# microsoft/CryptoNets

Measured on AMD Instinct MI355X. Metric: encrypted images/sec (CryptoNets-MNIST, N=8192), higher is better.
Workload: dtype u64

## Files before the change

### cryptonets_amd/csrc/cn_gemm_plan.h

```cpp
#pragma once
#include "cn_policy.h"
#include <algorithm>
#include <cstdio>
#include <cstdlib>
#include <cstring>
#include <map>
#include <type_traits>
#include <unordered_map>
#include <vector>

struct GemmSwitches { bool f64, gemm_mfma, gemm_pair, digit_mfma, digit_i32; };
static const int GEMM_ERR_ARG = -1;
struct GemmRefusal {
    int rc = 0; char msg[96] = {0};
    explicit operator bool() const { return rc != 0; }
};
inline GemmRefusal gemm_refuse(const char *text) { GemmRefusal r; r.rc = GEMM_ERR_ARG; snprintf(r.msg, sizeof r.msg, "%s", text); return r; }
inline size_t gemm_al(size_t b) { return (b + 255) & ~(size_t)255; }
static const uint32_t GEMM_NONE = 0xffffffffu;

inline uint64_t gemm_abs_weight(const DevConsts &hc, uint64_t w) { return w >= hc.t_half ? hc.t.q - w : w; }
inline uint64_t lift_scalar(const DevConsts &hc, uint64_t w, uint32_t j) { return w >= hc.t_half ? w + hc.lift_inc[j] : w; }
inline bool gemm_weights_small(const DevConsts &hc, const uint64_t *W, size_t count) {
    for (size_t x = 0; x < count; x++) if (gemm_abs_weight(hc, W[x]) >> 20) return false;
    return true;
}
struct GemmArith { bool small, two; uint32_t lazy; int bits; };
inline GemmArith gemm_arith(const DevConsts &hc, const GemmSwitches &sw, bool weights_small) {
    const CnModRange qr = cn_mod_range(hc, 0, hc.k);
    const int bits = qr.bits;
    GemmArith g;
    g.bits = bits;
    g.small = weights_small && sw.f64 && bits <= 49;
    g.two = qr.light;
    if (g.small) g.lazy = g.two ? 1024u : 32768u;
    else g.lazy = (2 * bits >= 127) ? 1u : (uint32_t)std::min<uint64_t>(1u << 20, 1ull << (127 - 2 * bits));
    return g;
}
inline bool gemm_mfma_ok(const DevConsts &hc, const GemmSwitches &sw, const GemmArith &ar, uint32_t M, uint32_t K) {
    return sw.gemm_mfma && ar.small && ar.bits <= 46 && M >= 16 && (uint64_t)K * 3 < (1u << 17) && !(hc.n & 31);
}
inline uint32_t gemm_weight_planes(const DevConsts &hc, const uint64_t *W, size_t count) {
    uint64_t amax = 0;
    for (size_t x = 0; x < count; x++) amax = std::max(amax, gemm_abs_weight(hc, W[x]));
    return amax <= 127 ? 1u : (amax <= 32639 ? 2u : 3u);
}

template <class KEY> inline std::map<std::vector<KEY>, std::vector<uint32_t>> gemm_outputs_by_list(const KEY *keys, uint32_t O, uint32_t K) {
    std::map<std::vector<KEY>, std::vector<uint32_t>> groups;
    for (uint32_t o = 0; o < O; o++) groups[std::vector<KEY>(keys + (size_t)o * K, keys + (size_t)(o + 1) * K)].push_back(o);
    return groups;
}
inline bool pair_gather_lists(uint32_t O, uint32_t &K, std::vector<int32_t> &gidx, const uint64_t *W, std::vector<uint64_t> &W2) {
    if (K > 64 || O < 2) return false;
    const auto groups = gemm_outputs_by_list(gidx.data(), O, K);
    const size_t G = groups.size();
    if (G < 2 || G > 65536) return false;
    struct L { std::vector<int32_t> in; const std::vector<uint32_t> *outs; const std::vector<int32_t> *list; int32_t mate = -1; };
    std::vector<L> ls; ls.reserve(G);
    for (auto &kv : groups) {
        if (kv.second.size() > 5) return false;
        L l; l.outs = &kv.second; l.list = &kv.first;
        for (int32_t id : kv.first) if (id >= 0) l.in.push_back(id);
        std::sort(l.in.begin(), l.in.end());
        if (std::adjacent_find(l.in.begin(), l.in.end()) != l.in.end()) return false;
        ls.push_back(std::move(l));
    }
    std::unordered_map<int32_t, std::vector<uint32_t>> where;
    for (uint32_t i = 0; i < G; i++) for (int32_t id : ls[i].in) where[id].push_back(i);
    bool any = false;
    std::vector<uint32_t> cnt(G, 0), touched;
    for (uint32_t i = 0; i < G; i++) {
        if (ls[i].mate >= 0) continue;
        touched.clear();
        for (int32_t id : ls[i].in) for (uint32_t j : where[id]) if (j > i && ls[j].mate < 0) { if (!cnt[j]++) touched.push_back(j); }
        uint32_t best = 0; int32_t bj = -1;
        for (uint32_t j : touched) { if (cnt[j] > best || (cnt[j] == best && (int32_t)j < bj)) { best = cnt[j]; bj = (int32_t)j; } cnt[j] = 0; }
        if (bj >= 0 && 2 * best >= std::min(ls[i].in.size(), ls[bj].in.size()) && ls[i].in.size() + ls[bj].in.size() - best <= 64) { ls[i].mate = bj; ls[bj].mate = (int32_t)i; any = true; }
    }
    if (!any) return false;
    std::vector<std::vector<int32_t>> uni(G);
    uint32_t K2 = 0;
    for (uint32_t i = 0; i < G; i++) {
        const int32_t m = ls[i].mate;
        if (m >= 0 && (uint32_t)m < i) { uni[i] = uni[m]; continue; }
        for (int32_t id : *ls[i].list) if (id >= 0) uni[i].push_back(id);
        if (m >= 0) for (int32_t id : *ls[m].list) if (id >= 0 && !std::binary_search(ls[i].in.begin(), ls[i].in.end(), id)) uni[i].push_back(id);
        K2 = std::max<uint32_t>(K2, (uint32_t)uni[i].size());
    }
    std::vector<int32_t> g2((size_t)O * K2, -1);
    W2.assign((size_t)O * K2, 0);
    for (uint32_t i = 0; i < G; i++) {
        std::unordered_map<int32_t, uint32_t> pos;
        for (uint32_t x = 0; x < uni[i].size(); x++) pos[uni[i][x]] = x;
        for (uint32_t o : *ls[i].outs) {
            for (uint32_t x = 0; x < uni[i].size(); x++) g2[(size_t)o * K2 + x] = uni[i][x];
            for (uint32_t kk = 0; kk < K; kk++) { const int32_t id = gidx[(size_t)o * K + kk]; if (id >= 0) W2[(size_t)o * K2 + pos[id]] = W[(size_t)o * K + kk]; }
        }
    }
    gidx.swap(g2); K = K2;
    return true;
}

template <class KEY> struct GemmGroups {
    static constexpr KEY PAD = std::is_signed<KEY>::value ? (KEY)-1 : (KEY)0;
    uint32_t O = 0, G = 0, M = 0, K = 0, Kp = 0;
    bool mfma = false;
    std::vector<KEY> rows;
    std::vector<uint32_t> member;
    const uint64_t *W = nullptr;
    bool tap(uint32_t g, uint32_t kk) const { return rows[(size_t)g * Kp + kk] > PAD; }
    const uint64_t *row(uint32_t g, uint32_t m) const { const uint32_t o = member[(size_t)g * M + m]; return o == GEMM_NONE ? nullptr : W + (size_t)o * K; }
    uint64_t weight(uint32_t g, const uint64_t *wr, uint32_t kk) const { return tap(g, kk) ? wr[kk] : 0; }
};
template <class KEY> inline GemmGroups<KEY> gemm_group(const DevConsts &hc, const GemmSwitches &sw, const GemmArith &ar, const KEY *keys, const uint64_t *W, uint32_t O, uint32_t K) {
    const auto groups = gemm_outputs_by_list(keys, O, K);
    GemmGroups<KEY> gr;
    gr.O = O; gr.G = (uint32_t)groups.size(); gr.K = K; gr.W = W;
    for (auto &g : groups) gr.M = std::max<uint32_t>(gr.M, (uint32_t)g.second.size());
    gr.mfma = gemm_mfma_ok(hc, sw, ar, gr.M, K);
    gr.Kp = gr.mfma ? ((K + 31) / 32) * 32 : ((K + 15) & ~15u) + 16;
    gr.rows.assign((size_t)gr.G * gr.Kp, GemmGroups<KEY>::PAD);
    gr.member.assign((size_t)gr.G * gr.M, GEMM_NONE);
    uint32_t g = 0;
    for (auto &kv : groups) {
        memcpy(&gr.rows[(size_t)g * gr.Kp], kv.first.data(), (size_t)K * sizeof(KEY));
        for (uint32_t m = 0; m < kv.second.size(); m++) gr.member[(size_t)g * gr.M + m] = kv.second[m];
        g++;
    }
    return gr;
}

template <class KEY> inline void pack_gemm_f64(const DevConsts &hc, const GemmGroups<KEY> &gr, uint32_t tile, uint32_t rows, std::vector<char> &bytes) {
    const uint32_t mt = (gr.M + tile - 1) / tile;
    bytes.assign((size_t)gr.G * mt * rows * tile * sizeof(double), 0);
    double *tab = (double *)bytes.data();
    for (uint32_t g = 0; g < gr.G; g++) for (uint32_t m = 0; m < gr.M; m++) {
        const uint64_t *wr = gr.row(g, m);
        if (!wr) continue;
        double *dst = &tab[(((size_t)g * mt + m / tile) * rows) * tile + m % tile];
        for (uint32_t kk = 0; kk < gr.K; kk++) { const uint64_t w = gr.weight(g, wr, kk); dst[(size_t)kk * tile] = w >= hc.t_half ? -(double)(hc.t.q - w) : (double)w; }
    }
}
template <class KEY> inline void pack_gemm_int(const DevConsts &hc, const GemmGroups<KEY> &gr, uint32_t tile, std::vector<char> &bytes) {
    const uint32_t mt = (gr.M + tile - 1) / tile, K = gr.K;
    bytes.assign((size_t)hc.k * gr.G * mt * K * tile * sizeof(uint64_t), 0);
    uint64_t *tab = (uint64_t *)bytes.data();
    for (uint32_t j = 0; j < hc.k; j++) for (uint32_t g = 0; g < gr.G; g++) for (uint32_t m = 0; m < gr.M; m++) {
        const uint64_t *wr = gr.row(g, m);
        if (!wr) continue;
        uint64_t *dst = &tab[((((size_t)j * gr.G + g) * mt + m / tile) * K) * tile + m % tile];
        for (uint32_t kk = 0; kk < K; kk++) { const uint64_t w = gr.weight(g, wr, kk); dst[(size_t)kk * tile] = w ? lift_scalar(hc, w, j) : 0; }
    }
}
template <class KEY> inline void pack_gemm_mfma(const DevConsts &hc, const GemmGroups<KEY> &gr, uint32_t P, std::vector<char> &wbytes) {
    const uint32_t mtiles = (gr.M + 31) / 32, ksteps = (gr.K + 31) / 32;
    const uint64_t t = hc.t.q;
    wbytes.assign((size_t)gr.G * P * mtiles * ksteps * 1024, 0);
    for (uint32_t g = 0; g < gr.G; g++) for (uint32_t m = 0; m < gr.M; m++) {
        const uint64_t *wr = gr.row(g, m);
        if (!wr) continue;
        const uint32_t mt = m / 32, r = m % 32;
        for (uint32_t kk = 0; kk < gr.K; kk++) {
            const uint64_t w = gr.weight(g, wr, kk);
            if (!w) continue;
            const int64_t sw = w >= hc.t_half ? -(int64_t)(t - w) : (int64_t)w;
            const uint32_t rec = ((uint32_t)(sw + 0x808080) ^ 0x808080u);
            const uint32_t ks = kk / 32, half = (kk % 32) / 16, tt = kk % 16;
            for (uint32_t p = 0; p < P; p++)
                wbytes[((((size_t)g * P + p) * mtiles + mt) * ksteps + ks) * 1024 + (size_t)(half * 32 + r) * 16 + tt] = (char)(uint8_t)(rec >> (8 * p));
        }
    }
}
template <class KEY> inline uint64_t gemm_row_sum_max(const DevConsts &hc, const GemmGroups<KEY> &gr, uint64_t stop) {
    uint64_t sum_max = 0;
    for (uint32_t g = 0; g < gr.G; g++) for (uint32_t m = 0; m < gr.M; m++) {
        const uint64_t *wr = gr.row(g, m);
        if (!wr) continue;
        uint64_t sum = 0;
        for (uint32_t kk = 0; kk < gr.K; kk++) if (gr.tap(g, kk)) { sum += gemm_abs_weight(hc, wr[kk]); if (sum > stop) return stop + 1; }
        sum_max = std::max(sum_max, sum);
    }
    return sum_max;
}
template <class KEY> inline bool gemm_one_limb(const DevConsts &hc, const GemmArith &ar, const GemmGroups<KEY> &gr) {
    static const bool on = !(getenv("CN_GEMM_ONE_LIMB") && !atoi(getenv("CN_GEMM_ONE_LIMB")));
    if (!on || !ar.small || ar.bits > 49 || gr.K > ar.lazy) return false;
    const uint64_t room = (1ull << 53) / cn_mod_range(hc, 0, hc.k).qmax;
    return room && gemm_row_sum_max(hc, gr, room - 1) <= room - 1;
}
template <class KEY> inline void gemm_form_and_pack(const DevConsts &hc, const GemmArith &ar, const GemmGroups<KEY> &gr, GemmLayout &L, std::vector<char> &wbytes) {
    const uint32_t M = gr.M;
    L.K = gr.K; L.Kp = gr.Kp; L.G = gr.G; L.M = M; L.small = ar.small; L.two = ar.two; L.lazy = ar.lazy; L.mfma = gr.mfma;
    if (gr.mfma) {
        L.P = gemm_weight_planes(hc, gr.W, (size_t)gr.O * gr.K); L.mtiles = (M + 31) / 32; L.ksteps = (gr.K + 31) / 32;
        pack_gemm_mfma(hc, gr, L.P, wbytes);
    } else if (ar.small) {
        L.MT = M >= 16 ? 20 : (M >= 8 ? 10 : (M >= 3 ? 5 : 1));
        pack_gemm_f64(hc, gr, L.MT, gemm_f64_rows(gr.K), wbytes);
        L.one = gemm_one_limb(hc, ar, gr);
    } else {
        L.MT = M >= 8 ? 10 : (M >= 3 ? 5 : 1);
        pack_gemm_int(hc, gr, L.MT, wbytes);
    }
}
template <class KEY> inline void gemm_digit_form(const DevConsts &hc, const GemmSwitches &sw, const GemmGroups<KEY> &gr, GemmLayout &L, std::vector<char> &dbytes) {
    if (!L.small || hc.k < 2 || hc.dbc < 1 || hc.dbc > 30) return;
    uint64_t qmin = ~0ull; for (uint32_t j = 0; j < hc.k; j++) qmin = std::min(qmin, hc.q[j].q);
    const uint64_t dmax = (1ull << hc.dbc) - 1, lim = std::min<uint64_t>((qmin - 1) / 2, (1ull << 52) - 1) / dmax;
    const uint64_t sum_max = gemm_row_sum_max(hc, gr, lim);
    if (sum_max > lim) return;
    L.dig = true; L.sum_abs_w = sum_max; L.dig_mfma = L.mfma && sw.digit_mfma && hc.dbc <= 14 && !(hc.n & 255); L.dig_i32 = sw.digit_i32 && cn_digit_sum_fits_i32(sum_max, hc.dbc);
    if (L.dig_mfma) return;
    L.dMT = digit_gemm_tile(L.M); L.dKw = digit_gemm_rows(L.K);
    pack_gemm_f64(hc, gr, L.dMT, L.dKw, dbytes);
}

template <class E> inline void gemm_assemble(const std::vector<E> &gather, const std::vector<E> &outs, const std::vector<E> &bias, const std::vector<char> &wbytes,
                                             const std::vector<char> &dbytes, GemmLayout &L, std::vector<char> &image) {
    L.off_oidx = gemm_al(gather.size() * sizeof(E)); L.off_bidx = L.off_oidx + gemm_al(outs.size() * sizeof(E)); L.off_w = L.off_bidx + gemm_al(bias.size() * sizeof(E));
    L.off_dw = L.off_w + gemm_al(wbytes.size());
    image.assign(L.off_dw + gemm_al(dbytes.size()), 0);
    if (!gather.empty()) memcpy(image.data(), gather.data(), gather.size() * sizeof(E));
    if (!outs.empty()) memcpy(image.data() + L.off_oidx, outs.data(), outs.size() * sizeof(E));
    if (!bias.empty()) memcpy(image.data() + L.off_bidx, bias.data(), bias.size() * sizeof(E));
    if (!wbytes.empty()) memcpy(image.data() + L.off_w, wbytes.data(), wbytes.size());
    if (!dbytes.empty()) memcpy(image.data() + L.off_dw, dbytes.data(), dbytes.size());
}

inline GemmRefusal gemm_plan_indices(const DevConsts &hc, const GemmSwitches &sw, const int32_t *idx, const uint64_t *W, uint32_t O, uint32_t K, const int32_t *bias_idx,
                                     uint32_t bias_count, GemmLayout &L, std::vector<char> &image, uint32_t &max_in, uint64_t &nnz) {
    if (!O || !K || !W) return gemm_refuse("empty scalar GEMM");
    std::vector<int32_t> gidx((size_t)O * K);
    for (uint32_t o = 0; o < O; o++) {
        bool any = false;
        for (uint32_t kk = 0; kk < K; kk++) {
            const int32_t id = idx ? idx[(size_t)o * K + kk] : (int32_t)kk;
            const uint64_t w = W[(size_t)o * K + kk];
            if (w >= hc.t.q) return gemm_refuse("weight >= plain modulus");
            if (id >= 0) max_in = std::max<uint32_t>(max_in, (uint32_t)id + 1);
            if (id >= 0 && w) { any = true; nnz++; }
            gidx[(size_t)o * K + kk] = id;
        }
        if (!any) { GemmRefusal r = gemm_refuse(""); snprintf(r.msg, sizeof r.msg, "output %u has no non-zero term (AddMany of nothing)", o); return r; }
        if (bias_idx && (bias_idx[o] < 0 || (uint32_t)bias_idx[o] >= bias_count)) return gemm_refuse("bias index out of range");
    }
    const GemmArith ar = gemm_arith(hc, sw, gemm_weights_small(hc, W, (size_t)O * K));
    std::vector<uint64_t> W2;
    if (sw.gemm_pair && ar.small && pair_gather_lists(O, K, gidx, W, W2)) W = W2.data();
    const GemmGroups<int32_t> gr = gemm_group(hc, sw, ar, gidx.data(), W, O, K);
    std::vector<int32_t> hoidx(gr.member.size(), -1), hbidx(gr.member.size(), 0);
    for (size_t x = 0; x < gr.member.size(); x++) if (gr.member[x] != GEMM_NONE) { hoidx[x] = (int32_t)gr.member[x]; if (bias_idx) hbidx[x] = bias_idx[gr.member[x]]; }
    std::vector<char> wbytes, dbytes;
    gemm_form_and_pack(hc, ar, gr, L, wbytes);
    gemm_digit_form(hc, sw, gr, L, dbytes);
    gemm_assemble(gr.rows, hoidx, hbidx, wbytes, dbytes, L, image);
    return GemmRefusal();
}
struct GemmAddressPlan {
    GemmLayout L; std::vector<char> image;
    bool abs = false, any_bias = false;
    uint64_t ibase = ~0ull, obase = ~0ull, bbase = ~0ull;
    uint64_t some_input = 0;
};
inline void gemm_plan_addresses(const DevConsts &hc, const GemmSwitches &sw, const uint64_t *A, const uint64_t *W, const uint64_t *out, const uint64_t *bias, uint32_t O, uint32_t K,
                                bool rel_on, GemmAddressPlan &R) {
    const GemmArith ar = gemm_arith(hc, sw, gemm_weights_small(hc, W, (size_t)O * K));
    const GemmGroups<uint64_t> gr = gemm_group(hc, sw, ar, A, W, O, K);
    std::vector<uint64_t> hoidx(gr.member.size(), 0), hbidx(gr.member.size(), 0);
    bool all_bias = true;
    for (size_t x = 0; x < gr.member.size(); x++) if (gr.member[x] != GEMM_NONE) {
        hoidx[x] = out[gr.member[x]]; hbidx[x] = bias[gr.member[x]];
        R.any_bias = R.any_bias || hbidx[x]; all_bias = all_bias && hbidx[x];
    }
    for (uint64_t a : gr.rows) if (a && !R.some_input) R.some_input = a;
    std::vector<char> wbytes;
    gemm_form_and_pack(hc, ar, gr, R.L, wbytes);
    bool rel = rel_on && (!R.any_bias || all_bias);
    if (rel) {
        for (uint64_t a : gr.rows) if (a) R.ibase = std::min(R.ibase, a);
        for (uint64_t a : hoidx) if (a) R.obase = std::min(R.obase, a);
        for (uint64_t a : hbidx) if (a) R.bbase = std::min(R.bbase, a);
        auto fits = [](uint64_t a, uint64_t base) { return !a || (((a - base) & 255) == 0 && ((a - base) >> 8) < 0x7fffffffull); };
        for (uint64_t a : gr.rows) rel = rel && fits(a, R.ibase);
        for (uint64_t a : hoidx) rel = rel && fits(a, R.obase);
        for (uint64_t a : hbidx) rel = rel && fits(a, R.bbase);
        rel = rel && R.ibase != ~0ull && R.obase != ~0ull;
    }
    R.abs = !rel;
    if (R.abs) { gemm_assemble(gr.rows, hoidx, hbidx, wbytes, {}, R.L, R.image); return; }
    auto relative = [](const std::vector<uint64_t> &a, uint64_t base, int32_t none) {
        std::vector<int32_t> r(a.size(), none);
        for (size_t x = 0; x < a.size(); x++) if (a[x]) r[x] = (int32_t)((a[x] - base) >> 8);
        return r;
    };
    gemm_assemble(relative(gr.rows, R.ibase, -1), relative(hoidx, R.obase, -1), relative(hbidx, R.bbase, 0), wbytes, {}, R.L, R.image);
}
```

### cryptonets_amd/csrc/cn_k_gemm.hip.h

```cpp
#pragma once
#include "cn_dev_common.hip.h"

DEV void gemm_block_coords(uint32_t bx, uint32_t by, uint32_t chunks, uint32_t limbs, uint32_t mtiles, uint32_t G, uint32_t &chunk, uint32_t &limb, uint32_t &mt, uint32_t &g,
                           uint32_t order = 0) {
    if (order == 1) {
        const uint32_t x = bx & 7, r = bx >> 3;
        if (mtiles == 1) { mt = 0; g = r; } else { mt = r % mtiles; g = r / mtiles; }
        const uint32_t sl = by * 8 + x;
        chunk = sl & (chunks - 1); limb = sl >> (__ffs((int)chunks) - 1);
        return;
    }
    const uint32_t b = bx, D = chunks * limbs * G;
    uint32_t d;
    if ((D & 7) == 0) { const uint32_t r = b >> 3; mt = r % mtiles; d = (r / mtiles) * 8 + (b & 7); }
    else { d = b % D; mt = b / D; }
    chunk = d % chunks; limb = (d / chunks) % limbs; g = d / (chunks * limbs);
}
DEV const NTT_GLOBAL uint64_t *gmem(uint64_t a) { return (const NTT_GLOBAL uint64_t *)a; }
DEV NTT_GLOBAL uint64_t *gmem_w(uint64_t a) { return (NTT_GLOBAL uint64_t *)a; }
struct GemmUnits { uint32_t in, out, bias; };
template <bool ABS> struct GemmTab { typedef int32_t T; };
template <> struct GemmTab<true> { typedef uint64_t T; };
template <int MT, bool ABS = false>
__global__ void __launch_bounds__(256) k_scalar_gemm(const uint64_t *__restrict__ in, const void *__restrict__ idx_, const uint64_t *__restrict__ Wl,
                                                     const void *__restrict__ out_idx_, const uint64_t *__restrict__ bias, const void *__restrict__ bias_idx_,
                                                     uint64_t *__restrict__ out, const DevConsts *__restrict__ C, uint32_t chunks, uint32_t G, uint32_t M,
                                                     uint32_t K, uint32_t mtiles, uint32_t lazy, uint32_t Kp, uint32_t obase, uint32_t polys, uint32_t order, GemmUnits U) {
    typedef typename GemmTab<ABS>::T TT;
    const TT *idx = (const TT *)idx_, *out_idx = (const TT *)out_idx_, *bias_idx = (const TT *)bias_idx_;
    const uint32_t n = C->n, k = C->k, limbs = polys * k;
    uint32_t chunk, limb, mt, g;
    gemm_block_coords(blockIdx.x, blockIdx.y, chunks, limbs, mtiles, G, chunk, limb, mt, g, order);
    const uint32_t j = limb % k, i = chunk * blockDim.x + threadIdx.x;
    const size_t ctw = (size_t)limbs * n, e = (size_t)limb * n + i;
    const size_t iu = U.in ? U.in : ctw, ou = U.out ? U.out : ctw, bu = U.bias ? U.bias : n;
    const DMod qm = C->q[j];
    u128 acc[MT];
#pragma unroll
    for (int m = 0; m < MT; m++) acc[m] = 0;
    const TT *gi = idx + (size_t)g * Kp;
    const uint64_t *gw = Wl + (((size_t)j * G + g) * mtiles + mt) * (size_t)K * MT;
    const uint32_t mcnt = min((uint32_t)MT, M - mt * MT);
    for (uint32_t k0 = 0; k0 < K; k0 += lazy) {
        const uint32_t k1 = min(K, k0 + lazy);
        for (uint32_t kk = k0; kk < k1; kk++) {
            uint64_t x;
            if constexpr (ABS) { const uint64_t a = gi[kk]; if (!a) continue; x = gmem(a)[e]; }
            else { const int32_t id = gi[kk]; if (id < 0) continue; x = in[(size_t)id * iu + e]; }
#pragma unroll
            for (int m = 0; m < MT; m++) acc[m] += (u128)x * gw[(size_t)kk * MT + m];
        }
        if (k1 < K) {
#pragma unroll
            for (int m = 0; m < MT; m++) acc[m] = bred128(acc[m], qm);
        }
    }
#pragma unroll
    for (int m = 0; m < MT; m++) {
        const uint32_t o = g * M + mt * MT + m;
        if constexpr (ABS) {
            if ((uint32_t)m < mcnt && out_idx[o]) {
                uint64_t r = bred128(acc[m], qm);
                if (bias_idx && bias_idx[o] && limb < k) { const uint64_t bv = gmem(bias_idx[o])[i]; if (bv) r = addmod(r, scale_plain(C, bv, j), qm.q); }
                gmem_w(out_idx[o])[e] = r;
            }
        } else if ((uint32_t)m < mcnt && out_idx[o] >= 0) {
            uint64_t r = bred128(acc[m], qm);
            if (bias && limb < k) { const uint64_t bv = bias[(size_t)bias_idx[o] * bu + i]; if (bv) r = addmod(r, scale_plain(C, bv, j), qm.q); }
            out[(size_t)(obase + (uint32_t)out_idx[o]) * ou + e] = r;
        }
    }
}

#ifndef GEMM_DPP_W
#define GEMM_DPP_W 1
#endif
template <int NL, int LW> DEV double gemm_limb(uint64_t x, int l) {
    if constexpr (NL == 1) return BzF::from_u64(x & 0x000FFFFFFFFFFFFFull);
    else return (double)(uint32_t)(l == NL - 1 ? x >> (l * LW) : (x >> (l * LW)) & ((1ull << LW) - 1));
}
template <int LANE> DEV void fmac_bcast(double &acc, double w, double x) {
    asm volatile("v_fmac_f64_dpp %0, %1, %2 row_newbcast:%3 row_mask:0xf bank_mask:0xf" : "+v"(acc) : "v"(w), "v"(x), "n"(LANE));
}
DEV void fmac_bcast_lane(int lane, double &acc, double w, double x) {
    switch (lane) {
    case 0: fmac_bcast<0>(acc, w, x); break;   case 1: fmac_bcast<1>(acc, w, x); break;   case 2: fmac_bcast<2>(acc, w, x); break;   case 3: fmac_bcast<3>(acc, w, x); break;
    case 4: fmac_bcast<4>(acc, w, x); break;   case 5: fmac_bcast<5>(acc, w, x); break;   case 6: fmac_bcast<6>(acc, w, x); break;   case 7: fmac_bcast<7>(acc, w, x); break;
    case 8: fmac_bcast<8>(acc, w, x); break;   case 9: fmac_bcast<9>(acc, w, x); break;   case 10: fmac_bcast<10>(acc, w, x); break; case 11: fmac_bcast<11>(acc, w, x); break;
    case 12: fmac_bcast<12>(acc, w, x); break; case 13: fmac_bcast<13>(acc, w, x); break; case 14: fmac_bcast<14>(acc, w, x); break; default: fmac_bcast<15>(acc, w, x); break;
    }
}
template <int MT, int NL, int LW, bool ABS = false>
__global__ void __launch_bounds__(256) k_scalar_gemm_f64(const uint64_t *__restrict__ in, const void *__restrict__ idx_, const double *__restrict__ Wd,
                                                         const void *__restrict__ out_idx_, const uint64_t *__restrict__ bias, const void *__restrict__ bias_idx_,
                                                         uint64_t *__restrict__ out, const DevConsts *__restrict__ C, uint32_t chunks, uint32_t G, uint32_t M,
                                                         uint32_t K, uint32_t mtiles, uint32_t lazy, uint32_t Kp, uint32_t obase, uint32_t polys, uint32_t order, uint32_t Kw, GemmUnits U) {
    typedef typename GemmTab<ABS>::T TT;
    const TT *idx = (const TT *)idx_, *out_idx = (const TT *)out_idx_, *bias_idx = (const TT *)bias_idx_;
    const uint32_t n = C->n, k = C->k, limbs = polys * k;
    uint32_t chunk, limb, mt, g;
    gemm_block_coords(blockIdx.x, blockIdx.y, chunks, limbs, mtiles, G, chunk, limb, mt, g, order);
    const uint32_t j = limb % k, i = chunk * blockDim.x + threadIdx.x;
    const size_t ctw = (size_t)limbs * n, e = (size_t)limb * n + i;
    const size_t iu = U.in ? U.in : ctw, ou = U.out ? U.out : ctw, bu = U.bias ? U.bias : n;
    const DMod qm = C->q[j];
    double acc[NL][MT], res[MT];
#pragma unroll
    for (int m = 0; m < MT; m++) {
        res[m] = 0.0;
#pragma unroll
        for (int l = 0; l < NL; l++) acc[l][m] = 0.0;
    }
    const TT *gi = idx + (size_t)g * Kp;
    const double *gw = Wd + ((size_t)g * mtiles + mt) * (size_t)Kw * MT;
    const uint32_t mcnt = min((uint32_t)MT, M - mt * MT);
    const BzF::Mod mq = {C->qd[j], C->qinvd[j]};
    auto fold = [&]() {
#pragma unroll
        for (int m = 0; m < MT; m++) {
            double r = acc[NL - 1][m];
            acc[NL - 1][m] = 0.0;
#pragma unroll
            for (int l = NL - 2; l >= 0; l--) { r = __dadd_rn(BzF::mulmod(r, (double)(1u << LW), mq), acc[l][m]); acc[l][m] = 0.0; }
            res[m] = BzF::center(__dadd_rn(res[m], r), mq);
        }
    };
#ifndef GEMM_PF_SMALL
#define GEMM_PF_SMALL 4
#endif
    constexpr int PF = (MT <= 5) ? GEMM_PF_SMALL : 4;
    static_assert(PF % 4 == 0, "gather indices travel in 16 B scalar loads of four");
    auto fetch = [&](uint64_t (&x)[PF], uint32_t kk) {
        const uint32_t kc = min(kk, Kp - PF);
        if constexpr (ABS) {
#pragma unroll
            for (int c = 0; c < PF; c += 4) {
                const ulonglong2 a01 = *reinterpret_cast<const ulonglong2 *>(__builtin_assume_aligned(gi + kc + c, 16));
                const ulonglong2 a23 = *reinterpret_cast<const ulonglong2 *>(__builtin_assume_aligned(gi + kc + c + 2, 16));
                const uint64_t ad[4] = {a01.x, a01.y, a23.x, a23.y};
#pragma unroll
                for (int p = 0; p < 4; p++) x[c + p] = gmem(ad[p] ? ad[p] : (uint64_t)in)[e];
            }
        } else {
#pragma unroll
            for (int c = 0; c < PF; c += 4) {
                const int4 ids = *reinterpret_cast<const int4 *>(__builtin_assume_aligned(gi + kc + c, 16));
                const int32_t id[4] = {ids.x, ids.y, ids.z, ids.w};
#pragma unroll
                for (int p = 0; p < 4; p++) x[c + p] = in[(size_t)max(id[p], 0) * iu + e];
            }
        }
    };
    constexpr int WB = MT >= 20 ? 1 : (MT * PF <= 20 ? PF : 20 / MT);
    constexpr bool WSET = WB == PF;
    auto wload = [&](double (&w)[WB * MT], uint32_t kk) {
        const double *wp = gw + (size_t)kk * MT;
#pragma unroll
        for (int q = 0; q < WB * MT; q++) w[q] = wp[q];
    };
    auto terms = [&](const uint64_t (&x)[PF], uint32_t kk, const double (&w0)[WB * MT]) {
#pragma unroll
        for (int p0 = 0; p0 < PF; p0 += WB) {
            double w[WB * MT];
            if constexpr (WSET) {
#pragma unroll
                for (int q = 0; q < WB * MT; q++) w[q] = w0[q];
            } else wload(w, kk + p0);
#pragma unroll
            for (int p = p0; p < p0 + WB; p++) {
                double xl[NL];
#pragma unroll
                for (int l = 0; l < NL; l++) xl[l] = gemm_limb<NL, LW>(x[p], l);
#pragma unroll
                for (int m = 0; m < MT; m++) {
#pragma unroll
                    for (int l = 0; l < NL; l++) acc[l][m] = __fma_rn(xl[l], w[(p - p0) * MT + m], acc[l][m]);
                }
            }
        }
    };
    constexpr bool DPPW = GEMM_DPP_W && MT == 20 && PF == 4;
    constexpr int WV = DPPW ? PF * MT / 16 : 1;
    auto wfetch = [&](double (&wv)[WV], uint32_t kk) {
        const double *wp = gw + (size_t)min(kk, K + 4) * MT + (threadIdx.x & 15);
#pragma unroll
        for (int v = 0; v < WV; v++) wv[v] = wp[16 * v];
    };
    auto terms_dpp = [&](const uint64_t (&x)[PF], double (&wv)[WV]) {
#pragma unroll
        for (int p = 0; p < PF; p++) {
            double xl[NL];
#pragma unroll
            for (int l = 0; l < NL; l++) xl[l] = gemm_limb<NL, LW>(x[p], l);
            asm volatile("s_nop 1");
#pragma unroll
            for (int m = 0; m < MT; m++) {
                const int f = p * MT + m;
#pragma unroll
                for (int l = 0; l < NL; l++) fmac_bcast_lane(f & 15, acc[l][m], wv[(f >> 4) % WV], xl[l]);
            }
        }
    };
    for (uint32_t k0 = 0; k0 < K; k0 += lazy) {
        const uint32_t k1 = min(K, k0 + lazy);
        uint64_t xa[PF], xb[PF];
        if constexpr (DPPW) {
            double wa[WV], wb[WV];
            fetch(xa, k0); wfetch(wa, k0);
            for (uint32_t kk = k0; kk < k1; kk += 2 * PF) {
                fetch(xb, kk + PF); wfetch(wb, kk + PF);
                terms_dpp(xa, wa);
                fetch(xa, kk + 2 * PF); wfetch(wa, kk + 2 * PF);
                terms_dpp(xb, wb);
            }
        } else {
            const uint32_t sets = (k1 - k0 + PF - 1) / PF;
            uint32_t kk = k0;
            double wa[WB * MT], wb[WB * MT];
            fetch(xa, k0);
            for (uint32_t it = sets >> 1; it; it--, kk += 2 * PF) {
                if constexpr (WSET) { wload(wa, kk); __builtin_amdgcn_sched_barrier(0); }
                fetch(xb, kk + PF);
                terms(xa, kk, wa);
                if constexpr (WSET) { wload(wb, kk + PF); __builtin_amdgcn_sched_barrier(0); }
                fetch(xa, kk + 2 * PF);
                terms(xb, kk + PF, wb);
            }
            if (sets & 1) { if constexpr (WSET) wload(wa, kk); terms(xa, kk, wa); }
        }
        fold();
    }
    constexpr int OB = MT < 5 ? MT : 5;
    const uint32_t olast = G * M - 1;
    const bool hb = (ABS ? bias_idx != nullptr : bias != nullptr) && limb < k;
#pragma unroll
    for (int m0 = 0; m0 < MT; m0 += OB) {
        uint32_t oo[OB];
        TT oi[OB], bi[OB];
        bool st[OB];
        uint64_t bv[OB];
#pragma unroll
        for (int u = 0; u < OB; u++) oo[u] = min(g * M + mt * MT + m0 + u, olast);
#pragma unroll
        for (int u = 0; u < OB; u++) { oi[u] = out_idx[oo[u]]; bi[u] = 0; bv[u] = 0; }
        if (hb) {
#pragma unroll
            for (int u = 0; u < OB; u++) bi[u] = bias_idx[oo[u]];
        }
#pragma unroll
        for (int u = 0; u < OB; u++) st[u] = (uint32_t)(m0 + u) < mcnt && (ABS ? oi[u] != 0 : (int64_t)oi[u] >= 0);
        if (hb) {
#pragma unroll
            for (int u = 0; u < OB; u++) {
                if constexpr (ABS) bv[u] = gmem(st[u] && bi[u] ? bi[u] : (uint64_t)in)[i];
                else bv[u] = bias[(size_t)(st[u] ? bi[u] : (TT)0) * bu + i];
            }
#pragma unroll
            for (int u = 0; u < OB; u++) if (!(st[u] && (ABS ? bi[u] != 0 : true))) bv[u] = 0;
        }
#pragma unroll
        for (int u = 0; u < OB; u++) {
            if (!st[u]) continue;
            const double rc = res[m0 + u] < 0.0 ? __dadd_rn(res[m0 + u], mq.q) : res[m0 + u];
            uint64_t r = (uint64_t)__double_as_longlong(__dadd_rn(rc, 4503599627370496.0)) & 0x000FFFFFFFFFFFFFull;
            if (bv[u]) r = addmod(r, scale_plain(C, bv[u], j), qm.q);
            if constexpr (ABS) gmem_w(oi[u])[e] = r;
            else out[(size_t)(obase + (uint32_t)oi[u]) * ou + e] = r;
        }
    }
}

typedef int v4i_t __attribute__((ext_vector_type(4)));
typedef int v16i_t __attribute__((ext_vector_type(16)));
DEV uint32_t byte_perm(uint32_t hi, uint32_t lo, uint32_t sel) { return __builtin_amdgcn_perm(hi, lo, sel); }
#ifndef GEMM_MFMA_DEPTH
#define GEMM_MFMA_DEPTH 2
#endif
enum { GEMM_CT = 0, GEMM_BSK = 1, GEMM_Y = 2 };
struct GemmBskForm { static constexpr int form = GEMM_BSK; };
struct GemmYForm { static constexpr int form = GEMM_Y; };
template <int P, bool ABS, class... FORM_>
__global__ void __launch_bounds__(256, 2) k_scalar_gemm_mfma(const uint64_t *__restrict__ in, const void *__restrict__ idx_, const int8_t *__restrict__ Wf,
                                                             const void *__restrict__ out_idx_, const uint64_t *__restrict__ bias, const void *__restrict__ bias_idx_,
                                                             uint64_t *__restrict__ out, const DevConsts *__restrict__ C, uint32_t G, uint32_t M, uint32_t mtiles,
                                                             uint32_t ksteps, uint32_t obase, uint32_t polys, GemmUnits U) {
    constexpr int FORM = (GEMM_CT + ... + FORM_::form);
    static_assert(sizeof...(FORM_) <= 1 && (FORM == GEMM_CT || !ABS), "the pre-floor forms use relative addressing");
    typedef typename GemmTab<ABS>::T TT;
    const TT *idx = (const TT *)idx_, *out_idx = (const TT *)out_idx_, *bias_idx = (const TT *)bias_idx_;
    constexpr int ND = FORM == GEMM_BSK ? 7 : 6, D = ND + P - 1, NB = GEMM_MFMA_DEPTH + 1;
    __shared__ __align__(16) uint32_t frag[NB][ND][64][4];
    const uint32_t n = C->n, k = FORM == GEMM_BSK ? C->kb : C->k, limbs = polys * k, ctiles = n >> 5;
    const uint32_t lane = threadIdx.x & 63, wave = (uint32_t)__builtin_amdgcn_readfirstlane((int)(threadIdx.x >> 6)), half = lane >> 5, col = lane & 31;
    uint32_t b = blockIdx.x;
    const uint32_t ctile = b % ctiles; b /= ctiles;
    const uint32_t limb = b % limbs; b /= limbs;
    const uint32_t mgroups = (mtiles + 3) >> 2, mg = b % mgroups, g = b / mgroups;
    const uint32_t mt = mg * 4 + wave;
    const bool active = mt < mtiles;
    const uint32_t j = limb % k;
    const size_t ctw = (size_t)limbs * n, e = (size_t)limb * n + (size_t)ctile * 32 + col;
    const size_t iu = U.in ? U.in : ctw, ou = U.out ? U.out : ctw, bu = U.bias ? U.bias : n;
    const uint32_t Kp = ksteps * 32;
    const TT *gi = idx + (size_t)g * Kp + 4 * wave;
    const int8_t *wf = Wf + ((((size_t)g * P) * mtiles + (active ? mt : 0)) * ksteps) * 1024 + (size_t)lane * 16;
    v16i_t acc[D];
#pragma unroll
    for (int d = 0; d < D; d++)
#pragma unroll
        for (int r = 0; r < 16; r++) acc[d][r] = 0;
    const uint64_t BIAS = FORM == GEMM_BSK ? 0x0080808080808080ull : 0x0000808080808080ull;
    const uint32_t klast = ksteps - 1;
    auto load_idx = [&](TT (&s)[8], uint32_t ks) {
        const TT *t = gi + (size_t)min(ks, klast) * 32;
#pragma unroll
        for (int u = 0; u < 4; u++) { s[u] = t[u]; s[4 + u] = t[16 + u]; }
    };
    auto load_x = [&](uint64_t (&x)[4], const TT (&s)[8]) {
#pragma unroll
        for (int u = 0; u < 4; u++) {
            if constexpr (ABS) {
                const uint64_t a0 = s[u] ? s[u] : (uint64_t)in, a1 = s[4 + u] ? s[4 + u] : (uint64_t)in;
                x[u] = gmem(half ? a1 : a0)[e];
            } else {
                size_t o0 = (size_t)max(s[u], 0) * iu, o1 = (size_t)max(s[4 + u], 0) * iu;
                asm volatile("" : "+s"(o0), "+s"(o1));
                x[u] = in[(half ? o1 : o0) + e];
            }
        }
    };
    auto load_a = [&](v4i_t (&af)[P], uint32_t ks) {
#pragma unroll
        for (int p = 0; p < P; p++) af[p] = *reinterpret_cast<const v4i_t *>(wf + ((size_t)p * mtiles * ksteps + min(ks, klast)) * 1024);
    };
    uint64_t xs[NB][4];
    v4i_t afs[NB][P];
    TT nidx[8];
    load_idx(nidx, 0);
#pragma unroll
    for (int s = 0; s < GEMM_MFMA_DEPTH; s++) { load_x(xs[s], nidx); load_a(afs[s], s); load_idx(nidx, s + 1); }
    auto step = [&](uint64_t (&x)[4], v4i_t (&af)[P], uint64_t (&xn)[4], v4i_t (&afn)[P], uint32_t ks, uint32_t (*fb)[64][4]) {
        uint32_t lo[4], hi[4];
#pragma unroll
        for (int u = 0; u < 4; u++) {
            uint64_t xw = x[u];
            if constexpr (FORM == GEMM_Y) {
                const BzF::Mod mq = {C->qd[j], C->qinvd[j]};
                const double yv = bz_canon(BzF::mulmod(lazy_value(xw), C->bd.fl_c1n_q[j], mq), mq);
                xw = (uint64_t)__double_as_longlong(__dadd_rn(yv, 4503599627370496.0)) & 0x000FFFFFFFFFFFFFull;
            }
            const uint64_t y = (xw + BIAS) ^ BIAS; lo[u] = (uint32_t)y; hi[u] = (uint32_t)(y >> 32);
        }
        const uint32_t ab02 = byte_perm(lo[1], lo[0], 0x06020400u), cd02 = byte_perm(lo[3], lo[2], 0x06020400u);
        const uint32_t ab13 = byte_perm(lo[1], lo[0], 0x07030501u), cd13 = byte_perm(lo[3], lo[2], 0x07030501u);
        const uint32_t hab = byte_perm(hi[1], hi[0], 0x05010400u), hcd = byte_perm(hi[3], hi[2], 0x05010400u);
        fb[0][lane][wave] = byte_perm(cd02, ab02, 0x05040100u);
        fb[1][lane][wave] = byte_perm(cd13, ab13, 0x05040100u);
        fb[2][lane][wave] = byte_perm(cd02, ab02, 0x07060302u);
        fb[3][lane][wave] = byte_perm(cd13, ab13, 0x07060302u);
        fb[4][lane][wave] = byte_perm(hcd, hab, 0x05040100u);
        fb[5][lane][wave] = byte_perm(hcd, hab, 0x07060302u);
        if constexpr (ND == 7) {
            const uint32_t hab6 = byte_perm(hi[1], hi[0], 0x06020602u), hcd6 = byte_perm(hi[3], hi[2], 0x06020602u);
            fb[ND - 1][lane][wave] = byte_perm(hcd6, hab6, 0x05040100u);
        }
        load_x(xn, nidx); load_a(afn, ks + GEMM_MFMA_DEPTH);
        load_idx(nidx, ks + GEMM_MFMA_DEPTH + 1);
        __syncthreads();
        if (active) {
            v4i_t bf[ND];
#pragma unroll
            for (int i = 0; i < ND; i++) bf[i] = *reinterpret_cast<const v4i_t *>(&fb[i][lane][0]);
#pragma unroll
            for (int p = 0; p < P; p++)
#pragma unroll
                for (int i = 0; i < ND; i++) acc[i + p] = __builtin_amdgcn_mfma_i32_32x32x32_i8(af[p], bf[i], acc[i + p], 0, 0, 0);
        }
    };
    uint32_t ks = 0;
    for (; ks + NB <= ksteps; ks += NB) {
#pragma unroll
        for (int s = 0; s < NB; s++) step(xs[s], afs[s], xs[(s + GEMM_MFMA_DEPTH) % NB], afs[(s + GEMM_MFMA_DEPTH) % NB], ks + s, frag[s]);
    }
#pragma unroll
    for (int s = 0; s < NB - 1; s++)
        if (ks + s < ksteps) step(xs[s], afs[s], xs[(s + GEMM_MFMA_DEPTH) % NB], afs[(s + GEMM_MFMA_DEPTH) % NB], ks + s, frag[s]);
    if (!active) return;
    if constexpr (FORM == GEMM_Y) {
#pragma unroll
        for (int r = 0; r < 16; r++) {
            const uint32_t row = (uint32_t)(r & 3) + 8u * (uint32_t)(r >> 2) + 4u * half, o = g * M + mt * 32 + row;
            if (mt * 32 + row >= M) continue;
            uint64_t v = 0;
#pragma unroll
            for (int d = 0; d < D; d++) v += (uint64_t)(int64_t)acc[d][r] << (8 * d);
            if (out_idx[o] < 0) continue;
            out[(size_t)(obase + (uint32_t)out_idx[o]) * ou + e] = v;
        }
        return;
    }
    const uint32_t jm = FORM == GEMM_BSK ? C->k + j : j;
    const BzF::Mod mq = {C->qd[jm], C->qinvd[jm]};
    const DMod qm = C->q[FORM == GEMM_BSK ? 0 : j];
    const double c24 = BzF::center(16777216.0, mq), c48 = BzF::center(__dmul_rn(c24, 16777216.0), mq);
#pragma unroll
    for (int r = 0; r < 16; r++) {
        const uint32_t row = (uint32_t)(r & 3) + 8u * (uint32_t)(r >> 2) + 4u * half, o = g * M + mt * 32 + row;
        if (mt * 32 + row >= M) continue;
        auto group = [&](int d0) {
            double t = (double)acc[d0][r];
            if (d0 + 1 < D) t = __fma_rn((double)acc[d0 + 1 < D ? d0 + 1 : d0][r], 256.0, t);
            if (d0 + 2 < D) t = __fma_rn((double)acc[d0 + 2 < D ? d0 + 2 : d0][r], 65536.0, t);
            return t;
        };
        double v = __dadd_rn(group(0), BzF::mulmod(group(3), c24, mq));
        if (D > 6) v = __dadd_rn(v, BzF::mulmod(group(6), c48, mq));
        uint64_t res = BzF::to_u64(v, mq);
        if constexpr (ABS) {
            if (!out_idx[o]) continue;
            if (bias_idx && bias_idx[o] && limb < k) { const uint64_t bv = gmem(bias_idx[o])[(size_t)ctile * 32 + col]; if (bv) res = addmod(res, scale_plain(C, bv, j), qm.q); }
            gmem_w(out_idx[o])[e] = res;
        } else {
            if (out_idx[o] < 0) continue;
            if (FORM == GEMM_CT && bias && limb < k) { const uint64_t bv = bias[(size_t)bias_idx[o] * bu + (size_t)ctile * 32 + col]; if (bv) res = addmod(res, scale_plain(C, bv, j), qm.q); }
            out[(size_t)(obase + (uint32_t)out_idx[o]) * ou + e] = res;
        }
    }
}

template <class... E> struct DigitWord { typedef double type; };
template <> struct DigitWord<int32_t> { typedef int32_t type; };
template <int MT, int DG, class... E>
__global__ void __launch_bounds__(256) k_digit_gemm(const uint64_t *__restrict__ in, size_t in_unit, const int32_t *__restrict__ idx, const double *__restrict__ Wd,
                                                    const int32_t *__restrict__ out_idx, typename DigitWord<E...>::type *__restrict__ S, const DevConsts *__restrict__ C, uint32_t G, uint32_t M,
                                                    uint32_t K, uint32_t mtiles, uint32_t Kp, uint32_t Kw, uint32_t ndg) {
    const uint32_t n = C->n, k = C->k, chunks = n >> 8;
    uint32_t chunk, lj, mt, g;
    gemm_block_coords(blockIdx.x, 0, chunks, k * ndg, mtiles, G, chunk, lj, mt, g);
    const uint32_t l = lj % k, d0 = (lj / k) * DG, nd = C->rl_dig[l];
    if (d0 >= nd) return;
    uint32_t g0 = 0;
    for (uint32_t x = 0; x < l; x++) g0 += C->rl_dig[x];
    const uint32_t i = chunk * 256 + threadIdx.x, dbc = (uint32_t)C->dbc, mask = (1u << dbc) - 1;
    const size_t e = (size_t)l * n + i;
    uint32_t sh[DG];
#pragma unroll
    for (int d = 0; d < DG; d++) sh[d] = min(dbc * (d0 + (uint32_t)d), 63u);
    double acc[DG][MT];
#pragma unroll
    for (int d = 0; d < DG; d++)
#pragma unroll
        for (int m = 0; m < MT; m++) acc[d][m] = 0.0;
    const int32_t *gi = idx + (size_t)g * Kp;
    const double *gw = Wd + ((size_t)g * mtiles + mt) * (size_t)Kw * MT;
    constexpr int PF = 4, WB = MT > 10 ? 1 : 2;
    auto fetch = [&](uint64_t (&x)[PF], uint32_t kk) {
        const int4 ids = *reinterpret_cast<const int4 *>(__builtin_assume_aligned(gi + min(kk, Kp - PF), 16));
        const int32_t id[4] = {ids.x, ids.y, ids.z, ids.w};
#pragma unroll
        for (int p = 0; p < PF; p++) x[p] = in[(size_t)max(id[p], 0) * in_unit + e];
    };
    auto terms = [&](const uint64_t (&x)[PF], uint32_t kk) {
#pragma unroll
        for (int p0 = 0; p0 < PF; p0 += WB) {
            double w[WB * MT];
            const double *wp = gw + (size_t)(kk + p0) * MT;
#pragma unroll
            for (int q = 0; q < WB * MT; q++) w[q] = wp[q];
#pragma unroll
            for (int p = p0; p < p0 + WB; p++) {
                double dg[DG];
#pragma unroll
                for (int d = 0; d < DG; d++) dg[d] = (double)((uint32_t)(x[p] >> sh[d]) & mask);
#pragma unroll
                for (int m = 0; m < MT; m++)
#pragma unroll
                    for (int d = 0; d < DG; d++) acc[d][m] = __fma_rn(dg[d], w[(p - p0) * MT + m], acc[d][m]);
            }
        }
    };
    {
        const uint32_t sets = (K + PF - 1) / PF;
        uint32_t kk = 0;
        uint64_t xa[PF], xb[PF];
        fetch(xa, 0);
        for (uint32_t it = sets >> 1; it; it--, kk += 2 * PF) {
            fetch(xb, kk + PF);
            terms(xa, kk);
            fetch(xa, kk + 2 * PF);
            terms(xb, kk + PF);
        }
        if (sets & 1) terms(xa, kk);
    }
    const uint32_t tot = C->rl_tot;
#pragma unroll
    for (int m = 0; m < MT; m++) {
        const uint32_t mm = mt * MT + (uint32_t)m;
        if (mm >= M) break;
        const int32_t o = out_idx[g * M + mm];
        if (o < 0) continue;
#pragma unroll
        for (int d = 0; d < DG; d++)
            if (d0 + (uint32_t)d < nd) S[((size_t)o * tot + g0 + d0 + (uint32_t)d) * n + i] = (typename DigitWord<E...>::type)acc[d][m];
    }
}

template <int P, int DG, class... E>
__global__ void __launch_bounds__(256, 2) k_digit_gemm_mfma(const uint64_t *__restrict__ in, size_t in_unit, const int32_t *__restrict__ idx, const int8_t *__restrict__ Wf,
                                                            const int32_t *__restrict__ out_idx, typename DigitWord<E...>::type *__restrict__ S, const DevConsts *__restrict__ C, uint32_t G,
                                                            uint32_t M, uint32_t mtiles, uint32_t ksteps, uint32_t ndg) {
    constexpr int NP = 2 * DG, D = P + 1, NB = GEMM_MFMA_DEPTH + 1;
    __shared__ __align__(16) uint32_t frag[NB][NP][64][4];
    const uint32_t n = C->n, k = C->k, ctiles = n >> 5;
    const uint32_t lane = threadIdx.x & 63, wave = (uint32_t)__builtin_amdgcn_readfirstlane((int)(threadIdx.x >> 6)), half = lane >> 5, col = lane & 31;
    uint32_t b = blockIdx.x;
    const uint32_t x8 = b & 7; b >>= 3;
    const uint32_t dgi = b % ndg; b /= ndg;
    const uint32_t ctile = (b % (ctiles >> 3)) * 8 + x8; b /= ctiles >> 3;
    const uint32_t l = b % k; b /= k;
    const uint32_t mgroups = (mtiles + 3) >> 2, mg = b % mgroups, g = b / mgroups;
    const uint32_t d0 = dgi * DG, nd = C->rl_dig[l];
    if (d0 >= nd) return;
    const uint32_t cnt = min((uint32_t)DG, nd - d0);
    uint32_t g0 = 0;
    for (uint32_t x = 0; x < l; x++) g0 += C->rl_dig[x];
    const uint32_t mt = mg * 4 + wave;
    const bool active = mt < mtiles;
    const uint32_t dbc = (uint32_t)C->dbc, mask = (1u << dbc) - 1;
    uint32_t sh[DG];
#pragma unroll
    for (int d = 0; d < DG; d++) sh[d] = min(dbc * (d0 + (uint32_t)d), 63u);
    const size_t e = (size_t)l * n + (size_t)ctile * 32 + col;
    const uint32_t Kp = ksteps * 32;
    const int32_t *gi = idx + (size_t)g * Kp + 4 * wave;
    const int8_t *wf = Wf + ((((size_t)g * P) * mtiles + (active ? mt : 0)) * ksteps) * 1024 + (size_t)lane * 16;
    v16i_t acc[DG][D];
#pragma unroll
    for (int d = 0; d < DG; d++)
#pragma unroll
        for (int j = 0; j < D; j++)
#pragma unroll
            for (int r = 0; r < 16; r++) acc[d][j][r] = 0;
    const uint32_t klast = ksteps - 1;
    auto load_idx = [&](int32_t (&s)[8], uint32_t ks) {
        const int32_t *t = gi + (size_t)min(ks, klast) * 32;
#pragma unroll
        for (int u = 0; u < 4; u++) { s[u] = t[u]; s[4 + u] = t[16 + u]; }
    };
    auto load_x = [&](uint64_t (&x)[4], const int32_t (&s)[8]) {
#pragma unroll
        for (int u = 0; u < 4; u++) {
            size_t o0 = (size_t)max(s[u], 0) * in_unit, o1 = (size_t)max(s[4 + u], 0) * in_unit;
            asm volatile("" : "+s"(o0), "+s"(o1));
            x[u] = in[(half ? o1 : o0) + e];
        }
    };
    auto load_a = [&](v4i_t (&af)[P], uint32_t ks) {
#pragma unroll
        for (int p = 0; p < P; p++) af[p] = *reinterpret_cast<const v4i_t *>(wf + ((size_t)p * mtiles * ksteps + min(ks, klast)) * 1024);
    };
    uint64_t xs[NB][4];
    v4i_t afs[NB][P];
    int32_t nidx[8];
    load_idx(nidx, 0);
#pragma unroll
    for (int s = 0; s < GEMM_MFMA_DEPTH; s++) { load_x(xs[s], nidx); load_a(afs[s], s); load_idx(nidx, s + 1); }
    auto step = [&](uint64_t (&x)[4], v4i_t (&af)[P], uint64_t (&xn)[4], v4i_t (&afn)[P], uint32_t ks, uint32_t (*fb)[64][4]) {
#pragma unroll
        for (int d = 0; d < DG; d++) {
            uint32_t t[4];
#pragma unroll
            for (int u = 0; u < 4; u++) t[u] = ((uint32_t)(x[u] >> sh[d]) & mask) + 128u;
            const uint32_t ab = byte_perm(t[1], t[0], 0x05010400u), cd = byte_perm(t[3], t[2], 0x05010400u);
            fb[2 * d][lane][wave] = byte_perm(cd, ab, 0x05040100u) ^ 0x80808080u;
            fb[2 * d + 1][lane][wave] = byte_perm(cd, ab, 0x07060302u);
        }
        load_x(xn, nidx); load_a(afn, ks + GEMM_MFMA_DEPTH);
        load_idx(nidx, ks + GEMM_MFMA_DEPTH + 1);
        __syncthreads();
        if (active) {
#pragma unroll
            for (int d = 0; d < DG; d++) {
                if ((uint32_t)d >= cnt) continue;
                const v4i_t blo = *reinterpret_cast<const v4i_t *>(&fb[2 * d][lane][0]), bhi = *reinterpret_cast<const v4i_t *>(&fb[2 * d + 1][lane][0]);
#pragma unroll
                for (int p = 0; p < P; p++) acc[d][p] = __builtin_amdgcn_mfma_i32_32x32x32_i8(af[p], blo, acc[d][p], 0, 0, 0);
#pragma unroll
                for (int p = 0; p < P; p++) acc[d][p + 1] = __builtin_amdgcn_mfma_i32_32x32x32_i8(af[p], bhi, acc[d][p + 1], 0, 0, 0);
            }
        }
    };
    uint32_t ks = 0;
    for (; ks + NB <= ksteps; ks += NB) {
#pragma unroll
        for (int s = 0; s < NB; s++) step(xs[s], afs[s], xs[(s + GEMM_MFMA_DEPTH) % NB], afs[(s + GEMM_MFMA_DEPTH) % NB], ks + s, frag[s]);
    }
#pragma unroll
    for (int s = 0; s < NB - 1; s++)
        if (ks + s < ksteps) step(xs[s], afs[s], xs[(s + GEMM_MFMA_DEPTH) % NB], afs[(s + GEMM_MFMA_DEPTH) % NB], ks + s, frag[s]);
    if (!active) return;
    const uint32_t tot = C->rl_tot, olast = G * M - 1;
    int32_t oo[16];
#pragma unroll
    for (int r = 0; r < 16; r++) {
        const uint32_t mm = mt * 32 + (uint32_t)(r & 3) + 8u * (uint32_t)(r >> 2) + 4u * half;
        oo[r] = out_idx[min(g * M + mm, olast)];
        if (mm >= M) oo[r] = -1;
    }
#pragma unroll
    for (int d = 0; d < DG; d++) {
        if ((uint32_t)d >= cnt) continue;
#pragma unroll
        for (int r = 0; r < 16; r++) {
            if (oo[r] < 0) continue;
            typename DigitWord<E...>::type *dst = S + ((size_t)oo[r] * tot + g0 + d0 + (uint32_t)d) * n + (size_t)ctile * 32 + col;
            if constexpr (std::is_same<typename DigitWord<E...>::type, int32_t>::value) {
                uint32_t v = (uint32_t)acc[d][D - 1][r];
#pragma unroll
                for (int j = D - 2; j >= 0; j--) v = (v << 8) + (uint32_t)acc[d][j][r];
                *dst = (int32_t)v;
            } else {
                double v = (double)acc[d][0][r];
#pragma unroll
                for (int j = 1; j < D; j++) v = __fma_rn((double)acc[d][j][r], (double)(1u << (8 * j)), v);
                *dst = v;
            }
        }
    }
}

typedef uint64_t ps_u64x2 __attribute__((ext_vector_type(2)));
typedef double ps_f64x2 __attribute__((ext_vector_type(2)));
DEV uint64_t ps_reduce(uint64_t x, const DMod &m) {
    const uint64_t r = x - __umul64hi(x, m.r1) * m.q;
    return r >= m.q ? r - m.q : r;
}
typedef int32_t ps_i32x2 __attribute__((ext_vector_type(2)));
template <int ND, class... E>
__global__ void __launch_bounds__(256) k_product_sum(const uint64_t *__restrict__ prod_, uint32_t K, uint64_t *__restrict__ out_, typename DigitWord<E...>::type *__restrict__ S_,
                                                     const DevConsts *__restrict__ C) {
    typedef const NTT_GLOBAL ps_u64x2 *In;
    constexpr int PF = 4;
    const uint32_t n = C->n, k = C->k, n2 = n >> 1, tiles = n >> 9;
    uint32_t b = blockIdx.x;
    const uint32_t tile = b % tiles; b /= tiles;
    const uint32_t l = b % k, o = b / k;
    const uint32_t p = tile * 256 + threadIdx.x;
    const uint32_t dbc = (uint32_t)C->dbc, mask = (1u << dbc) - 1, nd = C->rl_dig[l];
    uint32_t g0 = 0;
    for (uint32_t x = 0; x < l; x++) g0 += C->rl_dig[x];
    uint32_t sh[ND];
#pragma unroll
    for (int d = 0; d < ND; d++) sh[d] = min(dbc * (uint32_t)d, 63u);
    const size_t comp = (size_t)k * n2, unit = 3 * comp;
    const NTT_GLOBAL char *src = (const NTT_GLOBAL char *)prod_ + (size_t)o * K * unit * 16;
    const uint32_t lane_off = (l * n2 + p) * 16;
    uint64_t c0x = 0, c0y = 0, c1x = 0, c1y = 0, dx[ND], dy[ND];
#pragma unroll
    for (int d = 0; d < ND; d++) { dx[d] = 0; dy[d] = 0; }
    auto fetch = [&](ps_u64x2 (&x)[PF][3], uint32_t kk) {
#pragma unroll
        for (int t = 0; t < PF; t++) {
            const NTT_GLOBAL char *s = src + (size_t)min(kk + (uint32_t)t, K - 1) * unit * 16;
#pragma unroll
            for (int c = 0; c < 3; c++) x[t][c] = *(In)(s + (size_t)c * comp * 16 + lane_off);
        }
    };
    auto term = [&](const ps_u64x2 (&x)[3]) {
        c0x += x[0].x; c0y += x[0].y; c1x += x[1].x; c1y += x[1].y;
#pragma unroll
        for (int d = 0; d < ND; d++) { dx[d] += (uint32_t)(x[2].x >> sh[d]) & mask; dy[d] += (uint32_t)(x[2].y >> sh[d]) & mask; }
    };
    auto terms = [&](const ps_u64x2 (&x)[PF][3]) {
#pragma unroll
        for (int t = 0; t < PF; t++) term(x[t]);
    };
    auto tail = [&](const ps_u64x2 (&x)[PF][3], uint32_t nv) {
#pragma unroll
        for (int t = 0; t < PF; t++) if ((uint32_t)t < nv) term(x[t]);
    };
    {
        uint32_t kk = 0;
        ps_u64x2 xa[PF][3], xb[PF][3];
        fetch(xa, 0);
        for (uint32_t it = K / (2 * PF); it; it--, kk += 2 * PF) {
            fetch(xb, kk + PF);
            terms(xa);
            fetch(xa, kk + 2 * PF);
            terms(xb);
        }
        const uint32_t r = K - kk;
        if (r > PF) fetch(xb, kk + PF);
        tail(xa, min(r, (uint32_t)PF));
        if (r > PF) tail(xb, r - PF);
    }
    const DMod m = C->q[l];
    typedef NTT_GLOBAL ps_u64x2 *Out;
    Out dst = (Out)out_ + (size_t)o * 2 * comp + (size_t)l * n2 + p;
    ps_u64x2 v;
    v.x = ps_reduce(c0x, m); v.y = ps_reduce(c0y, m); dst[0] = v;
    v.x = ps_reduce(c1x, m); v.y = ps_reduce(c1y, m); dst[comp] = v;
    typedef typename DigitWord<E...>::type SE;
    typedef typename std::conditional<std::is_same<SE, int32_t>::value, ps_i32x2, ps_f64x2>::type SV;
    typedef NTT_GLOBAL SV *OutS;
    OutS sd = (OutS)S_ + ((size_t)o * C->rl_tot + g0) * n2 + p;
#pragma unroll
    for (int d = 0; d < ND; d++)
        if ((uint32_t)d < nd) { SV w; w.x = (SE)dx[d]; w.y = (SE)dy[d]; sd[(size_t)d * n2] = w; }
}
```

### cryptonets_amd/csrc/cn_l_gemm.hip

```cpp
#include "cn_runtime.h"
#include <algorithm>
#include "cn_k_gemm.hip.h"

struct GemmGrid { dim3 grid; uint32_t order; };
static GemmGrid gemm_grid(cn_ctx *c, const GemmLaunch &g, uint32_t mtiles) {
    const uint32_t slices = c->chunks * g.polys * c->hc.k;
    if (g.order == 1 && (slices & 7) == 0 && (c->chunks & (c->chunks - 1)) == 0 && (uint64_t)8 * mtiles * g.G < (1ull << 31) && slices / 8 < 65536)
        return {dim3(8 * mtiles * g.G, slices / 8), 1u};
    return {dim3((uint32_t)((size_t)slices * mtiles * g.G)), 0u};
}
template <int MT, bool ABS> static void launch_int(cn_ctx *c, const GemmLaunch &g) {
    const uint32_t mtiles = (g.M + MT - 1) / MT;
    const GemmGrid gg = gemm_grid(c, g, mtiles);
    hipLaunchKernelGGL((k_scalar_gemm<MT, ABS>), gg.grid, dim3(c->bs), 0, c->stream, g.in, g.idx, (const uint64_t *)g.W, g.oidx, g.bias, g.bidx, g.out, c->dc,
                       c->chunks, g.G, g.M, g.K, mtiles, g.lazy, g.Kp, g.obase, g.polys, gg.order, GemmUnits{g.in_unit, g.out_unit, g.bias_unit});
}
template <int MT, bool ABS> static void launch_f64(cn_ctx *c, const GemmLaunch &g) {
    const uint32_t mtiles = (g.M + MT - 1) / MT;
    const GemmGrid gg = gemm_grid(c, g, mtiles);
    if (g.one) hipLaunchKernelGGL((k_scalar_gemm_f64<MT, 1, 0, ABS>), gg.grid, dim3(c->bs), 0, c->stream, g.in, g.idx, (const double *)g.W, g.oidx, g.bias,
                                  g.bidx, g.out, c->dc, c->chunks, g.G, g.M, g.K, mtiles, g.lazy, g.Kp, g.obase, g.polys, gg.order, gemm_f64_rows(g.K), GemmUnits{g.in_unit, g.out_unit, g.bias_unit});
    else if (g.two) hipLaunchKernelGGL((k_scalar_gemm_f64<MT, 2, 22, ABS>), gg.grid, dim3(c->bs), 0, c->stream, g.in, g.idx, (const double *)g.W, g.oidx, g.bias,
                                  g.bidx, g.out, c->dc, c->chunks, g.G, g.M, g.K, mtiles, g.lazy, g.Kp, g.obase, g.polys, gg.order, gemm_f64_rows(g.K), GemmUnits{g.in_unit, g.out_unit, g.bias_unit});
    else hipLaunchKernelGGL((k_scalar_gemm_f64<MT, 3, 17, ABS>), gg.grid, dim3(c->bs), 0, c->stream, g.in, g.idx, (const double *)g.W, g.oidx, g.bias,
                            g.bidx, g.out, c->dc, c->chunks, g.G, g.M, g.K, mtiles, g.lazy, g.Kp, g.obase, g.polys, gg.order, gemm_f64_rows(g.K), GemmUnits{g.in_unit, g.out_unit, g.bias_unit});
}
template <bool ABS> static int launch(cn_ctx *c, const GemmLaunch &g) {
    if (g.small) {
        switch (g.MT) {
            case 20: launch_f64<20, ABS>(c, g); break;
            case 10: launch_f64<10, ABS>(c, g); break;
            case 5: launch_f64<5, ABS>(c, g); break;
            case 1: launch_f64<1, ABS>(c, g); break;
            default: return cn_fail(CN_ERR_ARG, "internal: scalar GEMM tile %u", g.MT);
        }
    } else {
        switch (g.MT) {
            case 10: launch_int<10, ABS>(c, g); break;
            case 5: launch_int<5, ABS>(c, g); break;
            case 1: launch_int<1, ABS>(c, g); break;
            default: return cn_fail(CN_ERR_ARG, "internal: scalar GEMM tile %u", g.MT);
        }
    }
    HIPCHK(hipGetLastError());
    cn_launch_count(c);
    return 0;
}
int cn_l_gemm(cn_ctx *c, const GemmLaunch &g) { return g.abs ? launch<true>(c, g) : launch<false>(c, g); }

template <int P, bool ABS> static void launch_mfma(cn_ctx *c, const GemmLaunch &g) {
    const uint32_t mgroups = (g.mtiles + 3) / 4;
    if constexpr (!ABS && P <= 2) {
        if (g.form) {
            const size_t pblocks = (size_t)g.G * mgroups * g.polys * (g.form == GEMM_BSK ? c->hc.kb : c->hc.k) * (c->hc.n / 32);
            if (g.form == GEMM_BSK) hipLaunchKernelGGL((k_scalar_gemm_mfma<P, false, GemmBskForm>), dim3((uint32_t)pblocks), dim3(256), 0, c->stream, g.in, g.idx, (const int8_t *)g.W, g.oidx,
                                                       nullptr, nullptr, g.out, c->dc, g.G, g.M, g.mtiles, g.ksteps, g.obase, g.polys, GemmUnits{g.in_unit, g.out_unit, 0u});
            else hipLaunchKernelGGL((k_scalar_gemm_mfma<P, false, GemmYForm>), dim3((uint32_t)pblocks), dim3(256), 0, c->stream, g.in, g.idx, (const int8_t *)g.W, g.oidx,
                                    nullptr, nullptr, g.out, c->dc, g.G, g.M, g.mtiles, g.ksteps, g.obase, g.polys, GemmUnits{g.in_unit, g.out_unit, 0u});
            return;
        }
    }
    const size_t blocks = (size_t)g.G * mgroups * g.polys * c->hc.k * (c->hc.n / 32);
    hipLaunchKernelGGL((k_scalar_gemm_mfma<P, ABS>), dim3((uint32_t)blocks), dim3(256), 0, c->stream, g.in, g.idx, (const int8_t *)g.W, g.oidx, g.bias, g.bidx, g.out,
                       c->dc, g.G, g.M, g.mtiles, g.ksteps, g.obase, g.polys, GemmUnits{g.in_unit, g.out_unit, g.bias_unit});
}
template <bool ABS> static int launch_mfma_p(cn_ctx *c, const GemmLaunch &g) {
    if (g.form && (ABS || g.P > 2 || g.form > GEMM_Y || !g.in_unit || !g.out_unit)) return cn_fail(CN_ERR_ARG, "internal: pre-floor GEMM form %u", g.form);
    switch (g.P) {
        case 1: launch_mfma<1, ABS>(c, g); break;
        case 2: launch_mfma<2, ABS>(c, g); break;
        case 3: launch_mfma<3, ABS>(c, g); break;
        default: return cn_fail(CN_ERR_ARG, "internal: %u weight digit planes", g.P);
    }
    HIPCHK(hipGetLastError());
    cn_launch_count(c);
    return 0;
}
int cn_l_gemm_mfma(cn_ctx *c, const GemmLaunch &g) { return g.abs ? launch_mfma_p<true>(c, g) : launch_mfma_p<false>(c, g); }

template <int MT> static void launch_digit(cn_ctx *c, const DigitGemmLaunch &g, uint32_t ndg, uint32_t mtiles) {
    const size_t blocks = (size_t)(c->hc.n >> 8) * c->hc.k * ndg * mtiles * g.G;
    if (g.i32) hipLaunchKernelGGL((k_digit_gemm<MT, 5, int32_t>), dim3((uint32_t)blocks), dim3(256), 0, c->stream, g.in, g.in_unit, (const int32_t *)g.idx, (const double *)g.W,
                                  (const int32_t *)g.oidx, (int32_t *)g.S, c->dc, g.G, g.M, g.K, mtiles, g.Kp, g.Kw, ndg);
    else hipLaunchKernelGGL((k_digit_gemm<MT, 5>), dim3((uint32_t)blocks), dim3(256), 0, c->stream, g.in, g.in_unit, (const int32_t *)g.idx, (const double *)g.W,
                            (const int32_t *)g.oidx, (double *)g.S, c->dc, g.G, g.M, g.K, mtiles, g.Kp, g.Kw, ndg);
}
template <int P, int DG> static void launch_digit_mfma(cn_ctx *c, const DigitGemmLaunch &g, uint32_t ndg, size_t blocks) {
    if (g.i32) hipLaunchKernelGGL((k_digit_gemm_mfma<P, DG, int32_t>), dim3((uint32_t)blocks), dim3(256), 0, c->stream, g.in, g.in_unit, (const int32_t *)g.idx, (const int8_t *)g.W,
                                  (const int32_t *)g.oidx, (int32_t *)g.S, c->dc, g.G, g.M, g.mtiles, g.ksteps, ndg);
    else hipLaunchKernelGGL((k_digit_gemm_mfma<P, DG>), dim3((uint32_t)blocks), dim3(256), 0, c->stream, g.in, g.in_unit, (const int32_t *)g.idx, (const int8_t *)g.W,
                            (const int32_t *)g.oidx, (double *)g.S, c->dc, g.G, g.M, g.mtiles, g.ksteps, ndg);
}
static int digit_gemm_mfma(cn_ctx *c, const DigitGemmLaunch &g, uint32_t ndmax) {
    const uint32_t DG = digit_gemm_mfma_group(g.P), ndg = (ndmax + DG - 1) / DG, mgroups = (g.mtiles + 3) / 4;
    const uint64_t blocks = (uint64_t)g.G * mgroups * c->hc.k * (c->hc.n / 32) * ndg;
    if ((c->hc.n & 255) || !g.ksteps || blocks >= (1ull << 31)) return cn_fail(CN_ERR_ARG, "internal: digit GEMM grid");
    switch (g.P) {
        case 1: launch_digit_mfma<1, 3>(c, g, ndg, blocks); break;
        case 2: launch_digit_mfma<2, 3>(c, g, ndg, blocks); break;
        case 3: launch_digit_mfma<3, 2>(c, g, ndg, blocks); break;
        default: return cn_fail(CN_ERR_ARG, "internal: %u weight digit planes", g.P);
    }
    HIPCHK(hipGetLastError());
    cn_launch_count(c);
    c->cnt.dg_mfma++;
    return 0;
}
int cn_l_digit_gemm(cn_ctx *c, const DigitGemmLaunch &g) {
    uint32_t ndmax = 0; for (uint32_t l = 0; l < c->hc.k; l++) ndmax = std::max(ndmax, c->hc.rl_dig[l]);
    if (g.mfma) return digit_gemm_mfma(c, g, ndmax);
    const uint32_t ndg = (ndmax + 4) / 5, mtiles = (g.M + g.MT - 1) / g.MT;
    if ((c->hc.n & 255) || (uint64_t)(c->hc.n >> 8) * c->hc.k * ndg * mtiles * g.G >= (1ull << 31)) return cn_fail(CN_ERR_ARG, "internal: digit GEMM grid");
    switch (g.MT) {
        case 10: launch_digit<10>(c, g, ndg, mtiles); break;
        case 2: launch_digit<2>(c, g, ndg, mtiles); break;
        default: return cn_fail(CN_ERR_ARG, "internal: digit GEMM tile %u", g.MT);
    }
    HIPCHK(hipGetLastError());
    cn_launch_count(c);
    return 0;
}

template <int ND> static void launch_product_sum(cn_ctx *c, const ProductSumLaunch &g, uint32_t blocks) {
    if (g.i32) hipLaunchKernelGGL((k_product_sum<ND, int32_t>), dim3(blocks), dim3(256), 0, c->stream, g.prod, g.K, g.out, (int32_t *)g.S, c->dc);
    else hipLaunchKernelGGL((k_product_sum<ND>), dim3(blocks), dim3(256), 0, c->stream, g.prod, g.K, g.out, (double *)g.S, c->dc);
}
int cn_l_product_sum(cn_ctx *c, const ProductSumLaunch &g) {
    uint32_t ndmax = 0; for (uint32_t l = 0; l < c->hc.k; l++) ndmax = std::max(ndmax, c->hc.rl_dig[l]);
    const uint64_t blocks = (uint64_t)(c->hc.n >> 9) * c->hc.k * g.outputs;
    if ((c->hc.n & 511) || !g.K || !g.outputs || ndmax > PRODUCT_SUM_MAX_DIGITS || c->hc.dbc > 31 || blocks >= (1ull << 31)) return cn_fail(CN_ERR_ARG, "internal: product sum grid");
    if (ndmax <= 2) launch_product_sum<2>(c, g, (uint32_t)blocks);
    else if (ndmax <= 4) launch_product_sum<4>(c, g, (uint32_t)blocks);
    else if (ndmax <= 5) launch_product_sum<5>(c, g, (uint32_t)blocks);
    else launch_product_sum<8>(c, g, (uint32_t)blocks);
    HIPCHK(hipGetLastError());
    cn_launch_count(c);
    return 0;
}
```

### cryptonets_amd/csrc/cn_policy.h

```cpp
#pragma once
#include "cn_internal.h"

enum { POL_U64 = 0, POL_F64 = 1, POL_F64L = 2 };

struct CnModRange {
    bool f64ok;
    bool light;
    int bits;
    uint64_t qmax;
};
inline CnModRange cn_mod_range(const DevConsts &hc, uint32_t base_off, uint32_t nmod) {
    CnModRange r{true, true, 0, 0};
    for (uint32_t m = base_off; m < base_off + nmod; m++) {
        const uint64_t q = m < hc.k ? hc.q[m].q : (m < hc.k + hc.kb ? hc.bsk[m - hc.k].q : hc.t.q);
        r.f64ok = r.f64ok && hc.f64ok[m];
        if (q > r.qmax) r.qmax = q;
    }
    r.light = !(r.qmax >> 44);
    r.bits = r.qmax ? 64 - __builtin_clzll(r.qmax) : 0;
    return r;
}
inline int cn_policy(const CnModRange &r, bool use_f64) { return !(use_f64 && r.f64ok) ? POL_U64 : (r.light ? POL_F64L : POL_F64); }
inline bool cn_digit_sum_fits_i32(uint64_t sum_abs_w, int dbc) {
    if (dbc < 1 || dbc > 31) return false;
    return (unsigned __int128)sum_abs_w * ((1ull << dbc) - 1) <= 0x7fffffffull;
}
inline bool cn_prefloor_bound_ok(uint64_t sum_abs_w, uint64_t t, uint32_t n, const uint64_t *q, uint32_t k, const uint64_t *base, uint32_t kb) {
    if (!sum_abs_w || !t || !n || !k || !kb) return false;
    double lhs = __builtin_log2((double)sum_abs_w) + __builtin_log2((double)t) + __builtin_log2((double)n) + 3.0, rhs = -1.0;
    for (uint32_t j = 0; j < k; j++) {
        if (!q[j] || (unsigned __int128)sum_abs_w * q[j] >= ((unsigned __int128)1 << 63)) return false;
        lhs += __builtin_log2((double)q[j]);
    }
    for (uint32_t b = 0; b < kb; b++) { if (base[b] < 2) return false; rhs += __builtin_log2((double)base[b]); }
    return lhs + 0x1p-20 <= rhs;
}
inline uint32_t gemm_f64_rows(uint32_t K) { return ((K + 15) & ~15u) + 16; }
inline uint32_t digit_gemm_tile(uint32_t M) { return M > 2 ? 10u : 2u; }
inline uint32_t digit_gemm_rows(uint32_t K) { return ((K + 7) & ~7u) + 8; }
struct GemmLayout {
    uint32_t K = 0, Kp = 0, G = 0, M = 0, MT = 0, lazy = 0;
    bool small = false, two = false, one = false, mfma = false;
    uint32_t P = 0, mtiles = 0, ksteps = 0;
    bool dig = false, dig_mfma = false, dig_i32 = false; uint32_t dMT = 0, dKw = 0;
    size_t off_oidx = 0, off_bidx = 0, off_w = 0, off_dw = 0;
    uint64_t sum_abs_w = 0;
    template <class E> const E *gather(const char *image) const { return (const E *)image; }
    template <class E> const E *members(const char *image) const { return (const E *)(image + off_oidx); }
};
static const uint32_t CN_PTN_INTERVAL_CAP = 1u << 16;
inline uint64_t cn_ptn_term_bound(uint64_t q) {
    const unsigned __int128 sq = (unsigned __int128)3 * q * q;
    return q / 2 + 1 + (uint64_t)((sq + (((unsigned __int128)1 << 53) - 1)) >> 53);
}
inline uint32_t cn_ptn_sum_interval(uint64_t qmax, bool *capped = nullptr) {
    const uint64_t fit = ((1ull << 52) - 1) / cn_ptn_term_bound(qmax);
    if (capped) *capped = fit > CN_PTN_INTERVAL_CAP;
    return fit > CN_PTN_INTERVAL_CAP ? CN_PTN_INTERVAL_CAP : (fit ? (uint32_t)fit : 1u);
}
constexpr bool cn_plain_wide(int policy, uint32_t logn) { return !(policy == POL_U64 && logn == 14); }
inline uint32_t cn_f64_acc_interval(int bits) { return bits >= 50 ? 1u : 1u << (50 - bits < 10 ? 50 - bits : 10); }
inline bool cn_rr_size(uint32_t logn, uint32_t max_logn = 14) { return logn >= 10 && logn <= max_logn; }
```

### cryptonets_amd/csrc/cn_runtime.h

```cpp
#pragma once
#include "../../include/cnhip.h"
#include "cn_policy.h"
#include "cn_options.h"
#include "cn_ks_plan.h"
#include "cn_mul_plan.h"
#include "cn_submit.h"
#include <hip/hip_runtime.h>
#include <atomic>
#include <cstring>
#include <map>
#include <memory>
#include <mutex>
#include <set>
#include <string>
#include <type_traits>
#include <unordered_map>
#include <vector>

int cn_fail(int code, const char *fmt, ...);
#define HIPCHK(x) do { hipError_t e_ = (x); if (e_ != hipSuccess) return cn_fail(CN_ERR_HIP, "%s failed: %s", #x, hipGetErrorString(e_)); } while (0)
#define CHECK(x) do { int rc_ = (x); if (rc_) return rc_; } while (0)

struct GemmPlan;
struct cn_ctx;
struct CapturedGraph {
    hipGraph_t graph = nullptr; hipGraphExec_t exec = nullptr;
    std::vector<std::unique_ptr<char[]>> staged;
    std::vector<std::pair<uint64_t *, size_t>> reserved;
    struct Member { cn_ctx *ctx; std::vector<std::pair<uint64_t *, size_t>> reserved; };
    std::vector<Member> members;
};
struct Buffer {
    int kind;
    std::shared_ptr<GemmPlan> plan;
    std::shared_ptr<CapturedGraph> cg;
    uint32_t count, size;
    uint64_t *d;
    size_t item_words;
    std::vector<uint8_t> pt_zero;
};
class HandleTable {
    struct Slot { Buffer b; uint32_t gen = 0; bool live = false; };
    std::vector<Slot> slots;
    std::vector<uint32_t> free_;
    size_t live_ = 0;
public:
    Buffer *find(cn_handle h) {
        const uint32_t s = (uint32_t)h - 1u;
        if ((uint32_t)h == 0 || s >= slots.size() || !slots[s].live || slots[s].gen != (uint32_t)(h >> 32)) return nullptr;
        return &slots[s].b;
    }
    cn_handle insert(Buffer &&b) {
        uint32_t s;
        if (!free_.empty()) { s = free_.back(); free_.pop_back(); } else { s = (uint32_t)slots.size(); slots.emplace_back(); }
        slots[s].b = std::move(b); slots[s].live = true; slots[s].gen = (slots[s].gen + 1) & 0x7fffffffu;
        live_++;
        return ((cn_handle)slots[s].gen << 32) | (cn_handle)(s + 1);
    }
    void erase(cn_handle h) {
        const uint32_t s = (uint32_t)h - 1u;
        slots[s].live = false; slots[s].b = Buffer(); free_.push_back(s); live_--;
    }
    size_t size() const { return live_; }
    template <class F> void for_each(F f) { for (Slot &s : slots) if (s.live) f(s.b); }
};
struct KsKey { uint64_t *d; bool owned; bool f64; };

struct CnReq {
    int (*fn)(void *) = nullptr; void *arg = nullptr; int rc = 0;
    std::atomic<int> done{0}, asleep{0};
    CnReq *next = nullptr;
    char err[256];
};
class CnMutex {
public:
    struct Node {};
    void lock(Node &n);
    void unlock(Node &n);
    template <class F> int run(F &&f) {
        if (!combining()) { Node n; lock(n); const int rc = f(); unlock(n); return rc; }
        if (try_take_me()) { const int rc = f(); serve(); release(); return rc; }
        typedef typename std::remove_reference<F>::type Fn;
        CnReq r;
        r.fn = [](void *p) -> int { return (*static_cast<Fn *>(p))(); };
        r.arg = (void *)&f; r.err[0] = 0;
        return submit(r);
    }
    bool try_lock() { return try_take_me(); }
    void unlock_now() { release(); }
    bool is_held() const { return held.load(std::memory_order_relaxed) != 0; }
private:
    std::atomic<int> held{0};
    std::atomic<int> spinners{0};
    std::atomic<int> sleepers{0}, wake_seq{0};
    std::atomic<uint32_t> last_owner{0}, burst{0};
    std::atomic<uint64_t> released_at{0};
    std::atomic<CnReq *> pending{nullptr};
    bool try_take(uint32_t me);
    bool try_take_me();
    static bool combining();
    void release();
    void serve();
    int submit(CnReq &r);
};
struct CnGuard {
    CnMutex &m; CnMutex::Node n;
    explicit CnGuard(CnMutex &m_) : m(m_) { m.lock(n); }
    ~CnGuard() { m.unlock(n); }
    CnGuard(const CnGuard &) = delete;
    CnGuard &operator=(const CnGuard &) = delete;
};

struct DeferQueue;
struct cn_ctx {
    int device = 0;
    hipStream_t stream = nullptr;
    CnTunables opt;
    DevConsts hc;
    DevConsts *dc = nullptr;
    uint64_t *tw = nullptr;
    CnMutex mu;
    HandleTable bufs;
    KsKey rlk{nullptr, false, false};
    double *twd = nullptr, *twdh = nullptr;
    std::map<uint64_t, KsKey> gk;
    uint64_t *sk = nullptr, *pk = nullptr;
    uint64_t rng_item = 0;
    uint32_t rng_key[8] = {0, 0, 0, 0, 0, 0, 0, 0};
    char *scratch = nullptr; size_t scap = 0, soff = 0, smax;
    std::vector<std::unique_ptr<char[]>> staged;
    cn_stats st{};
    hipEvent_t ev0 = nullptr, ev1 = nullptr;
    hipEvent_t ev_order = nullptr;
    uint32_t bs, chunks;
    std::vector<uint32_t> index_map;
    uint32_t *d_index_map = nullptr;
    size_t ctw2;
    std::unordered_map<size_t, std::vector<uint64_t *>> pool;
    size_t pool_bytes = 0, pool_max;
    void *slabs = nullptr;
    void *ks_part = nullptr; size_t ks_part_cap = 0;
    char *pin = nullptr, *pin_dev = nullptr; size_t pin_off = 0; uint32_t pin_laps = 0;
    char *stage = nullptr; size_t stage_cap = 0;
    int stream_tries = 0;
    std::atomic<int> probe_pins{0};
    std::atomic<bool> capturing{false};
    std::vector<std::unique_ptr<char[]>> cap_staged;
    std::vector<std::pair<uint64_t *, size_t>> cap_allocs;
    int graphs_alive = 0;
    cn_ctx *cap_root = nullptr;
    std::vector<cn_ctx *> cap_members;
    hipStream_t own_stream = nullptr;
    int member_graphs = 0;
    hipEvent_t ev_graph = nullptr;
    int cus = 0;
    CnCounters cnt;
    std::atomic<uint64_t> packed_bad{0};
    uint64_t ks_hoisted = 0;
    uint32_t ms_groups = 0;
    uint64_t uid = 0;
    hipStream_t stream2 = nullptr; hipEvent_t ev_fork = nullptr, ev_join = nullptr; bool stream2_failed = false;
    std::atomic<int> defer{0};
    DeferQueue *dq = nullptr;
    SubmitRing *ring = nullptr;
    ReadyRing *ready = nullptr;
    int async_rc = 0; std::string async_msg;
    bool level = false;
    bool rec_steps = false, rec_cols = false;
    std::set<int> rec_set;
    hipEvent_t ev_ms = nullptr;
    bool ms_f64 = false;
};

struct KsItem { const uint64_t *in; const void *key; uint32_t elt, pad; };
struct KsCall {
    const uint64_t *target = nullptr; size_t tstride = 0;
    const uint64_t *add0 = nullptr, *add1 = nullptr; size_t astride = 0;
    uint64_t *out = nullptr; uint32_t cnt = 0; int galois = 0;
    const uint64_t *extra = nullptr; size_t xstride = 0;
    uint64_t *const *out_tab = nullptr;
    const KsItem *items = nullptr;
    uint32_t perm_elt = 0;
    uint32_t next_elt = 0; uint64_t *next_out = nullptr;
    const void *dig = nullptr;
    bool dig_i32 = false;
    static KsCall relin(const uint64_t *prod, size_t kn, uint32_t cnt) {
        return {.target = prod + 2 * kn, .tstride = 3 * kn, .add0 = prod, .add1 = prod + kn, .astride = 3 * kn, .cnt = cnt};
    }
    static KsCall relin_digits(const void *S, bool i32, const uint64_t *base, size_t kn, uint32_t cnt) {
        return {.add0 = base, .add1 = base + kn, .astride = 2 * kn, .cnt = cnt, .dig = S, .dig_i32 = i32};
    }
    static KsCall galois_of(const uint64_t *c1, size_t c1_stride, const uint64_t *c0, size_t kn, uint32_t cnt) {
        return {.target = c1, .tstride = c1_stride, .add0 = c0, .astride = 2 * kn, .cnt = cnt, .galois = 1};
    }
    static KsCall galois_items(const KsItem *items, uint32_t cnt) { return {.cnt = cnt, .galois = 1, .items = items}; }
    KsCall &to(uint64_t *dense) { out = dense; return *this; }
    KsCall &to_table(uint64_t *const *tab) { out_tab = tab; return *this; }
    KsCall &plus(const uint64_t *acc, size_t stride) { extra = acc; xstride = stride; return *this; }
    KsCall &perm(uint32_t elt) { perm_elt = elt; return *this; }
    KsCall &next(uint32_t elt, uint64_t *nout) { next_elt = elt; next_out = nout; return *this; }
};
struct KsArgs : KsCall {
    const uint64_t *key;
    KsPlan plan;
};
struct FoldOut { uint64_t *out; uint32_t first, count; };
struct FoldTerm { double w; uint32_t enc, pad; };
struct RrOps {
    int (*set_attrs)(uint32_t logn, size_t lds);
    bool (*ntt)(cn_ctx *c, uint64_t *data, uint32_t limbs, uint32_t base_off, uint32_t nmod, int inverse);
    bool (*intt_tensor)(cn_ctx *c, const uint64_t *A, const uint64_t *B, uint64_t *D, uint32_t cnt, uint32_t base_off, uint32_t Lm, bool lazy);
    bool (*square_fused)(cn_ctx *c, const uint64_t *A, size_t astride, const uint64_t *const *atab, uint64_t *D, uint32_t cnt, uint32_t base_off, uint32_t Lm, const MulBase &b);
    bool (*mul_plain_fused)(cn_ctx *c, const uint64_t *pt, uint32_t pitch, uint32_t npt, uint64_t *lift, const uint64_t *src, size_t sstride, uint32_t pstride,
                            uint64_t *out, uint32_t count, uint32_t polys);
    bool (*enc_tail)(cn_ctx *c, const uint64_t *u, const uint64_t *pt, uint32_t pts, uint64_t *out, uint32_t cnt, const int8_t *noise, const void *tab);
    bool (*enc_fused)(cn_ctx *c, const int8_t *us, const uint64_t *pt, uint32_t pts, uint64_t *out, uint32_t cnt, const int8_t *noise, const void *tab);
    bool (*mul_plain_bcast)(cn_ctx *c, const uint64_t *pt, uint32_t pitch, const uint64_t *ctn, uint64_t *out, uint32_t count, uint32_t polys, uint32_t next_elt,
                            uint64_t *next_out, bool ptn);
    bool (*enc_fold)(cn_ctx *c, const int8_t *us, const int8_t *noise, const void *fout, const void *terms, uint32_t outputs);
};
struct KsHoistItem { const void *key; uint64_t *out; uint32_t elt, pad; };
struct KsHoistArgs { const uint64_t *in; const KsHoistItem *items; KsHoistPlan plan; };
struct KsOps {
    int (*set_attrs)(uint32_t logn, size_t lds);
    bool (*launch)(cn_ctx *c, const KsArgs &a);
    bool (*hoist)(cn_ctx *c, const KsHoistArgs &a);
};
extern const RrOps cn_rr_u64, cn_rr_f64, cn_rr_f64l;
extern const KsOps cn_ks_u64, cn_ks_f64, cn_ks_f64l;

int cn_l_behz_extend(cn_ctx *c, const uint64_t *src, uint32_t stride, const uint64_t *const *src_tab, uint64_t *aq, uint64_t *ab, uint32_t cnt, bool f64);
int cn_l_behz_floor(cn_ctx *c, const uint64_t *dq, const uint64_t *db, uint64_t *out, uint32_t cnt, bool f64, bool lazy);
int cn_l_behz_floor_c2(cn_ctx *c, const uint64_t *dq, const uint64_t *db, uint64_t *out, uint32_t cnt);
struct FloorOutLaunch { const uint64_t *X, *Y; const int32_t *oidx; const uint64_t *bias; const int32_t *bidx; uint64_t *out; uint32_t obase, slots; };
int cn_l_behz_floor_out(cn_ctx *c, const FloorOutLaunch &g);

struct GemmLaunch {
    bool small, two, abs; uint32_t MT;
    const uint64_t *in; const void *idx; const void *W; const void *oidx; const uint64_t *bias; const void *bidx; uint64_t *out;
    uint32_t G, M, K, lazy, Kp, obase;
    uint32_t P = 0, mtiles = 0, ksteps = 0;
    uint32_t polys = 2;
    uint32_t order = 0;
    bool one = false;
    uint32_t in_unit = 0, out_unit = 0, bias_unit = 0;
    uint32_t form = 0;
    static GemmLaunch of(const GemmLayout &L, const char *tables, uint32_t order) {
        return {.small = L.small, .two = L.two, .abs = false, .MT = L.MT, .in = nullptr, .idx = tables, .W = tables + L.off_w, .oidx = tables + L.off_oidx, .bias = nullptr,
                .bidx = tables + L.off_bidx, .out = nullptr, .G = L.G, .M = L.M, .K = L.K, .lazy = L.lazy, .Kp = L.Kp, .obase = 0, .P = L.P, .mtiles = L.mtiles, .ksteps = L.ksteps,
                .order = order, .one = L.one};
    }
    GemmLaunch &inputs(const uint64_t *base, uint32_t unit, uint32_t polys_) { in = base; in_unit = unit; polys = polys_; return *this; }
    GemmLaunch &gather(const void *rows) { idx = rows; return *this; }
    GemmLaunch &bias_at(const uint64_t *base, const void *entries, uint32_t unit) { bias = base; bidx = entries; bias_unit = unit; return *this; }
    GemmLaunch &outputs(uint64_t *base, uint32_t first, uint32_t unit) { out = base; obase = first; out_unit = unit; return *this; }
    GemmLaunch &prefloor(uint32_t form_) { form = form_; bias = nullptr; return *this; }
    GemmLaunch &addresses(const uint64_t *any, bool with_bias) { abs = true; in = any; if (!with_bias) bidx = nullptr; return *this; }
};
int cn_l_gemm(cn_ctx *c, const GemmLaunch &g);
int cn_l_gemm_mfma(cn_ctx *c, const GemmLaunch &g);
struct DigitGemmLaunch {
    const uint64_t *in; size_t in_unit; const void *idx; const void *W; const void *oidx; void *S;
    uint32_t G, M, K, Kp, Kw, MT;
    bool mfma = false; uint32_t P = 0, mtiles = 0, ksteps = 0;
    bool i32 = false;
    static DigitGemmLaunch of(const GemmLayout &L, const char *tables, const uint64_t *in, size_t in_unit, const void *idx, void *S) {
        return {.in = in, .in_unit = in_unit, .idx = idx, .W = tables + (L.dig_mfma ? L.off_w : L.off_dw), .oidx = tables + L.off_oidx, .S = S, .G = L.G, .M = L.M, .K = L.K,
                .Kp = L.Kp, .Kw = L.dKw, .MT = L.dMT, .mfma = L.dig_mfma, .P = L.dig_mfma ? L.P : 0, .mtiles = L.dig_mfma ? L.mtiles : 0, .ksteps = L.dig_mfma ? L.ksteps : 0,
                .i32 = L.dig_i32};
    }
};
inline uint32_t digit_gemm_mfma_group(uint32_t P) { return P <= 2 ? 3u : 2u; }
int cn_l_digit_gemm(cn_ctx *c, const DigitGemmLaunch &g);
struct ProductSumLaunch { const uint64_t *prod; uint32_t K; uint64_t *out; void *S; uint32_t outputs; bool i32 = false; };
int cn_l_product_sum(cn_ctx *c, const ProductSumLaunch &g);
struct MulPlainSumLaunch { const uint64_t *pt, *ctn; const uint32_t *grp_off, *slot; uint64_t *out; uint32_t groups, accmax, order; };
int cn_l_mul_plain_sum(cn_ctx *c, int policy, const MulPlainSumLaunch &a);
int cn_l_diag_set_attrs(uint32_t logn, size_t lds);
int cn_l_mul_ptn_sum(cn_ctx *c, int policy, const MulPlainSumLaunch &a);
int cn_l_ptn_set_attrs(uint32_t logn, size_t lds);
struct DiagRunHost { uint32_t c, J, b0, len, first; };
static const uint32_t CN_DIAG_RUN = 32, CN_DIAG_MAX_RUNS = 65535;
int cn_l_diag_scan(cn_ctx *c, const uint64_t *S, uint32_t R, uint32_t dim, uint8_t *flags);
int cn_l_diag_gather(cn_ctx *c, const uint64_t *S, uint32_t R, uint32_t dim, const DiagRunHost *runs, uint32_t nruns, const uint32_t *index_map, uint64_t *out, uint8_t *nz);
int cn_l_mod_switch(cn_ctx *c, const uint64_t *src, uint64_t *dst, const DevConsts *src_consts, uint32_t ks, uint32_t kd, uint32_t items, uint32_t logn,
                    bool f64, bool *ran_f64);
int cn_l_noise_norm(cn_ctx *c, const uint64_t *c0, size_t ct_stride, const uint64_t *acc, uint64_t *out, uint32_t count);
int cn_l_crt_join(cn_ctx *c, const uint64_t *plain, const uint32_t *index_map, const void *tab, uint32_t P, uint32_t W, double *values, uint64_t *words, uint32_t count, uint32_t nslots);
int cn_l_join_argmax(cn_ctx *c, const uint64_t *words, uint32_t W, int32_t *argmax, uint32_t count, uint32_t nslots);
int cn_l_crt_split(cn_ctx *c, const void *values, int64_t stride_ct, int64_t stride_slot, uint32_t count, uint32_t nvalues, uint32_t flags, double scale,
                   const uint64_t *t, uint64_t *const *dst, uint32_t P, const uint32_t *index_map, uint32_t *nz, uint32_t nz_stride, uint32_t *bad);
struct SeededArgs {
    uint64_t *out; size_t ct_stride; uint32_t cnt; bool expand_only;
    const uint8_t *a_seed32; uint64_t a_nonce, a_item0;
    const int8_t *noise; const uint64_t *pt; uint32_t pt_stride_words;
};
int cn_l_seeded(cn_ctx *c, const SeededArgs &a);
size_t cn_packed_row_words(const cn_ctx *c);
int cn_l_unpack_rows(cn_ctx *c, const uint64_t *packed, uint64_t *arr, size_t item_words, uint32_t cnt, uint32_t polys, uint32_t *flag, hipStream_t stream = nullptr);
int cn_l_pack_rows(cn_ctx *c, const uint64_t *arr, size_t item_words, uint64_t *packed, uint32_t cnt, uint32_t polys, hipStream_t stream = nullptr);
struct KskGenArgs {
    const void *outs, *fac; const uint16_t *perm; const int8_t *noise;
    uint64_t seed, item0; uint32_t elts, tot; bool f64out;
};
int cn_l_ksk_gen(cn_ctx *c, const KskGenArgs &a);

inline void cn_launch_count(cn_ctx *c, int n = 1) { c->st.kernel_launches += n; }
```

Baseline: 1.334 million.

## Split weights into clipped int8 plane plus sparse residual k-steps for MFMA GEMM

When the largest weight magnitude is between 128 and 254, the MFMA GEMM now uses a single int8 plane with weights clipped to ±127. The leftover residual goes into a second plane, and only the K-columns holding large weights are reordered to the front. The kernel runs extra k-steps just over those residual columns instead of doubling every k-step with a second plane. This cuts MFMA work and weight traffic when few columns have large weights. The cost is a column permutation, a per-group residual count, and tighter overflow limits on the digit path. It is on by default through CN_GEMM_RESIDUAL.

After: 1.378 million, median of 6. 3.3% higher.

```diff
diff --git a/cryptonets_amd/csrc/cn_gemm_plan.h b/cryptonets_amd/csrc/cn_gemm_plan.h
--- a/cryptonets_amd/csrc/cn_gemm_plan.h
+++ b/cryptonets_amd/csrc/cn_gemm_plan.h
@@ -40,6 +40,7 @@
 inline bool gemm_mfma_ok(const DevConsts &hc, const GemmSwitches &sw, const GemmArith &ar, uint32_t M, uint32_t K) {
     return sw.gemm_mfma && ar.small && ar.bits <= 46 && M >= 16 && (uint64_t)K * 3 < (1u << 17) && !(hc.n & 31);
 }
+static const uint64_t GEMM_RES_CLIP = 127, GEMM_RES_MAX = 254;
 inline uint32_t gemm_weight_planes(const DevConsts &hc, const uint64_t *W, size_t count) {
     uint64_t amax = 0;
     for (size_t x = 0; x < count; x++) amax = std::max(amax, gemm_abs_weight(hc, W[x]));
@@ -109,9 +110,12 @@
     std::vector<KEY> rows;
     std::vector<uint32_t> member;
     const uint64_t *W = nullptr;
+    bool res = false;
+    std::vector<uint32_t> src, kres;
+    uint32_t term(uint32_t g, uint32_t kk) const { return src.empty() ? kk : src[(size_t)g * K + kk]; }
     bool tap(uint32_t g, uint32_t kk) const { return rows[(size_t)g * Kp + kk] > PAD; }
     const uint64_t *row(uint32_t g, uint32_t m) const { const uint32_t o = member[(size_t)g * M + m]; return o == GEMM_NONE ? nullptr : W + (size_t)o * K; }
-    uint64_t weight(uint32_t g, const uint64_t *wr, uint32_t kk) const { return tap(g, kk) ? wr[kk] : 0; }
+    uint64_t weight(uint32_t g, const uint64_t *wr, uint32_t kk) const { return tap(g, kk) ? wr[term(g, kk)] : 0; }
 };
 template <class KEY> inline GemmGroups<KEY> gemm_group(const DevConsts &hc, const GemmSwitches &sw, const GemmArith &ar, const KEY *keys, const uint64_t *W, uint32_t O, uint32_t K) {
     const auto groups = gemm_outputs_by_list(keys, O, K);
@@ -156,7 +160,9 @@
 template <class KEY> inline void pack_gemm_mfma(const DevConsts &hc, const GemmGroups<KEY> &gr, uint32_t P, std::vector<char> &wbytes) {
     const uint32_t mtiles = (gr.M + 31) / 32, ksteps = (gr.K + 31) / 32;
     const uint64_t t = hc.t.q;
-    wbytes.assign((size_t)gr.G * P * mtiles * ksteps * 1024, 0);
+    const size_t frags = (size_t)gr.G * P * mtiles * ksteps * 1024;
+    wbytes.assign(frags + (gr.res ? gr.G * sizeof(uint32_t) : 0), 0);
+    if (gr.res) memcpy(wbytes.data() + frags, gr.kres.data(), gr.G * sizeof(uint32_t));
     for (uint32_t g = 0; g < gr.G; g++) for (uint32_t m = 0; m < gr.M; m++) {
         const uint64_t *wr = gr.row(g, m);
         if (!wr) continue;
@@ -165,7 +171,9 @@
             const uint64_t w = gr.weight(g, wr, kk);
             if (!w) continue;
             const int64_t sw = w >= hc.t_half ? -(int64_t)(t - w) : (int64_t)w;
-            const uint32_t rec = ((uint32_t)(sw + 0x808080) ^ 0x808080u);
+            const int64_t cl = std::min<int64_t>(std::max<int64_t>(sw, -(int64_t)GEMM_RES_CLIP), (int64_t)GEMM_RES_CLIP);
+            const uint32_t rec = gr.res ? ((uint32_t)(uint8_t)(int8_t)cl | (uint32_t)(uint8_t)(int8_t)(sw - cl) << 8)
+                                        : ((uint32_t)(sw + 0x808080) ^ 0x808080u);
             const uint32_t ks = kk / 32, half = (kk % 32) / 16, tt = kk % 16;
             for (uint32_t p = 0; p < P; p++)
                 wbytes[((((size_t)g * P + p) * mtiles + mt) * ksteps + ks) * 1024 + (size_t)(half * 32 + r) * 16 + tt] = (char)(uint8_t)(rec >> (8 * p));
@@ -178,10 +186,41 @@
         const uint64_t *wr = gr.row(g, m);
         if (!wr) continue;
         uint64_t sum = 0;
-        for (uint32_t kk = 0; kk < gr.K; kk++) if (gr.tap(g, kk)) { sum += gemm_abs_weight(hc, wr[kk]); if (sum > stop) return stop + 1; }
+        for (uint32_t kk = 0; kk < gr.K; kk++) if (gr.tap(g, kk)) { sum += gemm_abs_weight(hc, wr[gr.term(g, kk)]); if (sum > stop) return stop + 1; }
         sum_max = std::max(sum_max, sum);
     }
     return sum_max;
+}
+static const uint32_t GEMM_RES_SHARE = 8;
+inline int gemm_residual_mode() { const char *e = getenv("CN_GEMM_RESIDUAL"); return e ? std::min(std::max(atoi(e), 0), 2) : 1; }
+template <class KEY> inline void gemm_residual_form(const DevConsts &hc, GemmGroups<KEY> &gr) {
+    const int mode = gemm_residual_mode();
+    if (!gr.mfma || !mode) return;
+    uint64_t amax = 0;
+    for (size_t x = 0; x < (size_t)gr.O * gr.K; x++) amax = std::max(amax, gemm_abs_weight(hc, gr.W[x]));
+    if (amax <= GEMM_RES_CLIP || amax > GEMM_RES_MAX) return;
+    const uint32_t K = gr.K, ksteps = (K + 31) / 32;
+    const uint64_t stop = ((1ull << 31) - 1) / 128;
+    if (gemm_row_sum_max(hc, gr, stop) > stop) return;
+    std::vector<uint32_t> src((size_t)gr.G * K), kres(gr.G);
+    for (uint32_t g = 0; g < gr.G; g++) {
+        std::vector<uint8_t> big(K, 0);
+        for (uint32_t m = 0; m < gr.M; m++) {
+            const uint64_t *wr = gr.row(g, m);
+            if (wr) for (uint32_t kk = 0; kk < K; kk++) if (gr.tap(g, kk) && gemm_abs_weight(hc, wr[kk]) > GEMM_RES_CLIP) big[kk] = 1;
+        }
+        uint32_t at = 0;
+        for (uint32_t kk = 0; kk < K; kk++) if (big[kk]) src[(size_t)g * K + at++] = kk;
+        kres[g] = (at + 31) / 32;
+        if ((mode == 2 ? 2 : GEMM_RES_SHARE) * kres[g] > ksteps) return;
+        for (uint32_t kk = 0; kk < K; kk++) if (!big[kk]) src[(size_t)g * K + at++] = kk;
+    }
+    std::vector<KEY> row(K);
+    for (uint32_t g = 0; g < gr.G; g++) {
+        for (uint32_t kk = 0; kk < K; kk++) row[kk] = gr.rows[(size_t)g * gr.Kp + src[(size_t)g * K + kk]];
+        std::copy(row.begin(), row.end(), gr.rows.begin() + (size_t)g * gr.Kp);
+    }
+    gr.res = true; gr.src.swap(src); gr.kres.swap(kres);
 }
 template <class KEY> inline bool gemm_one_limb(const DevConsts &hc, const GemmArith &ar, const GemmGroups<KEY> &gr) {
     static const bool on = !(getenv("CN_GEMM_ONE_LIMB") && !atoi(getenv("CN_GEMM_ONE_LIMB")));
@@ -193,8 +232,9 @@
     const uint32_t M = gr.M;
     L.K = gr.K; L.Kp = gr.Kp; L.G = gr.G; L.M = M; L.small = ar.small; L.two = ar.two; L.lazy = ar.lazy; L.mfma = gr.mfma;
     if (gr.mfma) {
-        L.P = gemm_weight_planes(hc, gr.W, (size_t)gr.O * gr.K); L.mtiles = (M + 31) / 32; L.ksteps = (gr.K + 31) / 32;
-        pack_gemm_mfma(hc, gr, L.P, wbytes);
+        L.P = gr.res ? 1 : gemm_weight_planes(hc, gr.W, (size_t)gr.O * gr.K); L.mtiles = (M + 31) / 32; L.ksteps = (gr.K + 31) / 32;
+        L.res = gr.res;
+        pack_gemm_mfma(hc, gr, gr.res ? 2 : L.P, wbytes);
     } else if (ar.small) {
         L.MT = M >= 16 ? 20 : (M >= 8 ? 10 : (M >= 3 ? 5 : 1));
         pack_gemm_f64(hc, gr, L.MT, gemm_f64_rows(gr.K), wbytes);
@@ -210,7 +250,7 @@
     const uint64_t dmax = (1ull << hc.dbc) - 1, lim = std::min<uint64_t>((qmin - 1) / 2, (1ull << 52) - 1) / dmax;
     const uint64_t sum_max = gemm_row_sum_max(hc, gr, lim);
     if (sum_max > lim) return;
-    L.dig = true; L.sum_abs_w = sum_max; L.dig_mfma = L.mfma && sw.digit_mfma && hc.dbc <= 14 && !(hc.n & 255); L.dig_i32 = sw.digit_i32 && cn_digit_sum_fits_i32(sum_max, hc.dbc);
+    L.dig = true; L.sum_abs_w = sum_max; L.dig_mfma = L.mfma && sw.digit_mfma && hc.dbc <= 14 && !(hc.n & 255) && (!L.res || sum_max * (128 + 64) < (1ull << 31)); L.dig_i32 = sw.digit_i32 && cn_digit_sum_fits_i32(sum_max, hc.dbc);
     if (L.dig_mfma) return;
     L.dMT = digit_gemm_tile(L.M); L.dKw = digit_gemm_rows(L.K);
     pack_gemm_f64(hc, gr, L.dMT, L.dKw, dbytes);
@@ -248,7 +288,8 @@
     const GemmArith ar = gemm_arith(hc, sw, gemm_weights_small(hc, W, (size_t)O * K));
     std::vector<uint64_t> W2;
     if (sw.gemm_pair && ar.small && pair_gather_lists(O, K, gidx, W, W2)) W = W2.data();
-    const GemmGroups<int32_t> gr = gemm_group(hc, sw, ar, gidx.data(), W, O, K);
+    GemmGroups<int32_t> gr = gemm_group(hc, sw, ar, gidx.data(), W, O, K);
+    gemm_residual_form(hc, gr);
     std::vector<int32_t> hoidx(gr.member.size(), -1), hbidx(gr.member.size(), 0);
     for (size_t x = 0; x < gr.member.size(); x++) if (gr.member[x] != GEMM_NONE) { hoidx[x] = (int32_t)gr.member[x]; if (bias_idx) hbidx[x] = bias_idx[gr.member[x]]; }
     std::vector<char> wbytes, dbytes;
@@ -266,7 +307,8 @@
 inline void gemm_plan_addresses(const DevConsts &hc, const GemmSwitches &sw, const uint64_t *A, const uint64_t *W, const uint64_t *out, const uint64_t *bias, uint32_t O, uint32_t K,
                                 bool rel_on, GemmAddressPlan &R) {
     const GemmArith ar = gemm_arith(hc, sw, gemm_weights_small(hc, W, (size_t)O * K));
-    const GemmGroups<uint64_t> gr = gemm_group(hc, sw, ar, A, W, O, K);
+    GemmGroups<uint64_t> gr = gemm_group(hc, sw, ar, A, W, O, K);
+    gemm_residual_form(hc, gr);
     std::vector<uint64_t> hoidx(gr.member.size(), 0), hbidx(gr.member.size(), 0);
     bool all_bias = true;
     for (size_t x = 0; x < gr.member.size(); x++) if (gr.member[x] != GEMM_NONE) {
diff --git a/cryptonets_amd/csrc/cn_k_gemm.hip.h b/cryptonets_amd/csrc/cn_k_gemm.hip.h
--- a/cryptonets_amd/csrc/cn_k_gemm.hip.h
+++ b/cryptonets_amd/csrc/cn_k_gemm.hip.h
@@ -277,15 +277,19 @@
 #define GEMM_MFMA_DEPTH 2
 #endif
 enum { GEMM_CT = 0, GEMM_BSK = 1, GEMM_Y = 2 };
-struct GemmBskForm { static constexpr int form = GEMM_BSK; };
-struct GemmYForm { static constexpr int form = GEMM_Y; };
+struct GemmBskForm { static constexpr int form = GEMM_BSK; static constexpr bool res = false; };
+struct GemmYForm { static constexpr int form = GEMM_Y; static constexpr bool res = false; };
+struct GemmResidual { static constexpr int form = GEMM_CT; static constexpr bool res = true; };
 template <int P, bool ABS, class... FORM_>
 __global__ void __launch_bounds__(256, 2) k_scalar_gemm_mfma(const uint64_t *__restrict__ in, const void *__restrict__ idx_, const int8_t *__restrict__ Wf,
                                                              const void *__restrict__ out_idx_, const uint64_t *__restrict__ bias, const void *__restrict__ bias_idx_,
                                                              uint64_t *__restrict__ out, const DevConsts *__restrict__ C, uint32_t G, uint32_t M, uint32_t mtiles,
                                                              uint32_t ksteps, uint32_t obase, uint32_t polys, GemmUnits U) {
     constexpr int FORM = (GEMM_CT + ... + FORM_::form);
-    static_assert(sizeof...(FORM_) <= 1 && (FORM == GEMM_CT || !ABS), "the pre-floor forms use relative addressing");
+    constexpr bool RES = (false || ... || FORM_::res);
+    constexpr int PW = RES ? 2 : P;
+    static_assert(sizeof...(FORM_) <= (RES ? 2 : 1) && FORM <= GEMM_Y && (FORM == GEMM_CT || !ABS), "the pre-floor forms use relative addressing");
+    static_assert(!RES || P == 1, "clipped + residual weights: one plane and its residual");
     typedef typename GemmTab<ABS>::T TT;
     const TT *idx = (const TT *)idx_, *out_idx = (const TT *)out_idx_, *bias_idx = (const TT *)bias_idx_;
     constexpr int ND = FORM == GEMM_BSK ? 7 : 6, D = ND + P - 1, NB = GEMM_MFMA_DEPTH + 1;
@@ -303,7 +307,7 @@
     const size_t iu = U.in ? U.in : ctw, ou = U.out ? U.out : ctw, bu = U.bias ? U.bias : n;
     const uint32_t Kp = ksteps * 32;
     const TT *gi = idx + (size_t)g * Kp + 4 * wave;
-    const int8_t *wf = Wf + ((((size_t)g * P) * mtiles + (active ? mt : 0)) * ksteps) * 1024 + (size_t)lane * 16;
+    const int8_t *wf = Wf + ((((size_t)g * PW) * mtiles + (active ? mt : 0)) * ksteps) * 1024 + (size_t)lane * 16;
     v16i_t acc[D];
 #pragma unroll
     for (int d = 0; d < D; d++)
@@ -311,8 +315,13 @@
         for (int r = 0; r < 16; r++) acc[d][r] = 0;
     const uint64_t BIAS = FORM == GEMM_BSK ? 0x0080808080808080ull : 0x0000808080808080ull;
     const uint32_t klast = ksteps - 1;
+    uint32_t kres = 0;
+    if constexpr (RES) kres = reinterpret_cast<const uint32_t *>(Wf + (size_t)G * PW * mtiles * ksteps * 1024)[g];
+    const uint32_t vsteps = RES ? ksteps + kres : ksteps;
+    auto kstep = [&](uint32_t v) { if constexpr (RES) { const uint32_t vv = min(v, vsteps - 1); return vv < kres ? vv : vv - kres; } else return min(v, klast); };
+    auto fragment = [&](uint32_t v) { if constexpr (RES) return min(v, vsteps - 1) < kres ? mtiles * ksteps + kstep(v) : kstep(v); else return min(v, klast); };
     auto load_idx = [&](TT (&s)[8], uint32_t ks) {
-        const TT *t = gi + (size_t)min(ks, klast) * 32;
+        const TT *t = gi + (size_t)kstep(ks) * 32;
 #pragma unroll
         for (int u = 0; u < 4; u++) { s[u] = t[u]; s[4 + u] = t[16 + u]; }
     };
@@ -331,7 +340,7 @@
     };
     auto load_a = [&](v4i_t (&af)[P], uint32_t ks) {
 #pragma unroll
-        for (int p = 0; p < P; p++) af[p] = *reinterpret_cast<const v4i_t *>(wf + ((size_t)p * mtiles * ksteps + min(ks, klast)) * 1024);
+        for (int p = 0; p < P; p++) af[p] = *reinterpret_cast<const v4i_t *>(wf + ((size_t)p * mtiles * ksteps + fragment(ks)) * 1024);
     };
     uint64_t xs[NB][4];
     v4i_t afs[NB][P];
@@ -378,13 +387,13 @@
         }
     };
     uint32_t ks = 0;
-    for (; ks + NB <= ksteps; ks += NB) {
+    for (; ks + NB <= vsteps; ks += NB) {
 #pragma unroll
         for (int s = 0; s < NB; s++) step(xs[s], afs[s], xs[(s + GEMM_MFMA_DEPTH) % NB], afs[(s + GEMM_MFMA_DEPTH) % NB], ks + s, frag[s]);
     }
 #pragma unroll
     for (int s = 0; s < NB - 1; s++)
-        if (ks + s < ksteps) step(xs[s], afs[s], xs[(s + GEMM_MFMA_DEPTH) % NB], afs[(s + GEMM_MFMA_DEPTH) % NB], ks + s, frag[s]);
+        if (ks + s < vsteps) step(xs[s], afs[s], xs[(s + GEMM_MFMA_DEPTH) % NB], afs[(s + GEMM_MFMA_DEPTH) % NB], ks + s, frag[s]);
     if (!active) return;
     if constexpr (FORM == GEMM_Y) {
 #pragma unroll
@@ -430,6 +439,8 @@
 
 template <class... E> struct DigitWord { typedef double type; };
 template <> struct DigitWord<int32_t> { typedef int32_t type; };
+template <> struct DigitWord<GemmResidual> { typedef double type; };
+template <> struct DigitWord<int32_t, GemmResidual> { typedef int32_t type; };
 template <int MT, int DG, class... E>
 __global__ void __launch_bounds__(256) k_digit_gemm(const uint64_t *__restrict__ in, size_t in_unit, const int32_t *__restrict__ idx, const double *__restrict__ Wd,
                                                     const int32_t *__restrict__ out_idx, typename DigitWord<E...>::type *__restrict__ S, const DevConsts *__restrict__ C, uint32_t G, uint32_t M,
@@ -505,11 +516,15 @@
     }
 }
 
+constexpr int DIGIT_GEMM_RES_GROUP = 5;
 template <int P, int DG, class... E>
 __global__ void __launch_bounds__(256, 2) k_digit_gemm_mfma(const uint64_t *__restrict__ in, size_t in_unit, const int32_t *__restrict__ idx, const int8_t *__restrict__ Wf,
                                                             const int32_t *__restrict__ out_idx, typename DigitWord<E...>::type *__restrict__ S, const DevConsts *__restrict__ C, uint32_t G,
                                                             uint32_t M, uint32_t mtiles, uint32_t ksteps, uint32_t ndg) {
     constexpr int NP = 2 * DG, D = P + 1, NB = GEMM_MFMA_DEPTH + 1;
+    constexpr bool RES = (false || ... || std::is_same<E, GemmResidual>::value);
+    constexpr int PW = RES ? 2 : P;
+    static_assert(!RES || P == 1, "clipped + residual weights: one plane and its residual");
     __shared__ __align__(16) uint32_t frag[NB][NP][64][4];
     const uint32_t n = C->n, k = C->k, ctiles = n >> 5;
     const uint32_t lane = threadIdx.x & 63, wave = (uint32_t)__builtin_amdgcn_readfirstlane((int)(threadIdx.x >> 6)), half = lane >> 5, col = lane & 31;
@@ -533,7 +548,7 @@
     const size_t e = (size_t)l * n + (size_t)ctile * 32 + col;
     const uint32_t Kp = ksteps * 32;
     const int32_t *gi = idx + (size_t)g * Kp + 4 * wave;
-    const int8_t *wf = Wf + ((((size_t)g * P) * mtiles + (active ? mt : 0)) * ksteps) * 1024 + (size_t)lane * 16;
+    const int8_t *wf = Wf + ((((size_t)g * PW) * mtiles + (active ? mt : 0)) * ksteps) * 1024 + (size_t)lane * 16;
     v16i_t acc[DG][D];
 #pragma unroll
     for (int d = 0; d < DG; d++)
@@ -542,8 +557,13 @@
 #pragma unroll
             for (int r = 0; r < 16; r++) acc[d][j][r] = 0;
     const uint32_t klast = ksteps - 1;
+    uint32_t kres = 0;
+    if constexpr (RES) kres = reinterpret_cast<const uint32_t *>(Wf + (size_t)G * PW * mtiles * ksteps * 1024)[g];
+    const uint32_t vsteps = RES ? ksteps + kres : ksteps;
+    auto kstep = [&](uint32_t v) { if constexpr (RES) { const uint32_t vv = min(v, vsteps - 1); return vv < kres ? vv : vv - kres; } else return min(v, klast); };
+    auto fragment = [&](uint32_t v) { if constexpr (RES) return min(v, vsteps - 1) < kres ? mtiles * ksteps + kstep(v) : kstep(v); else return min(v, klast); };
     auto load_idx = [&](int32_t (&s)[8], uint32_t ks) {
-        const int32_t *t = gi + (size_t)min(ks, klast) * 32;
+        const int32_t *t = gi + (size_t)kstep(ks) * 32;
 #pragma unroll
         for (int u = 0; u < 4; u++) { s[u] = t[u]; s[4 + u] = t[16 + u]; }
     };
@@ -557,7 +577,7 @@
     };
     auto load_a = [&](v4i_t (&af)[P], uint32_t ks) {
 #pragma unroll
-        for (int p = 0; p < P; p++) af[p] = *reinterpret_cast<const v4i_t *>(wf + ((size_t)p * mtiles * ksteps + min(ks, klast)) * 1024);
+        for (int p = 0; p < P; p++) af[p] = *reinterpret_cast<const v4i_t *>(wf + ((size_t)p * mtiles * ksteps + fragment(ks)) * 1024);
     };
     uint64_t xs[NB][4];
     v4i_t afs[NB][P];
@@ -591,13 +611,13 @@
         }
     };
     uint32_t ks = 0;
-    for (; ks + NB <= ksteps; ks += NB) {
+    for (; ks + NB <= vsteps; ks += NB) {
 #pragma unroll
         for (int s = 0; s < NB; s++) step(xs[s], afs[s], xs[(s + GEMM_MFMA_DEPTH) % NB], afs[(s + GEMM_MFMA_DEPTH) % NB], ks + s, frag[s]);
     }
 #pragma unroll
     for (int s = 0; s < NB - 1; s++)
-        if (ks + s < ksteps) step(xs[s], afs[s], xs[(s + GEMM_MFMA_DEPTH) % NB], afs[(s + GEMM_MFMA_DEPTH) % NB], ks + s, frag[s]);
+        if (ks + s < vsteps) step(xs[s], afs[s], xs[(s + GEMM_MFMA_DEPTH) % NB], afs[(s + GEMM_MFMA_DEPTH) % NB], ks + s, frag[s]);
     if (!active) return;
     const uint32_t tot = C->rl_tot, olast = G * M - 1;
     int32_t oo[16];
diff --git a/cryptonets_amd/csrc/cn_l_gemm.hip b/cryptonets_amd/csrc/cn_l_gemm.hip
--- a/cryptonets_amd/csrc/cn_l_gemm.hip
+++ b/cryptonets_amd/csrc/cn_l_gemm.hip
@@ -48,26 +48,27 @@
 }
 int cn_l_gemm(cn_ctx *c, const GemmLaunch &g) { return g.abs ? launch<true>(c, g) : launch<false>(c, g); }
 
-template <int P, bool ABS> static void launch_mfma(cn_ctx *c, const GemmLaunch &g) {
+template <int P, bool ABS, class... RES> static void launch_mfma(cn_ctx *c, const GemmLaunch &g) {
     const uint32_t mgroups = (g.mtiles + 3) / 4;
     if constexpr (!ABS && P <= 2) {
         if (g.form) {
             const size_t pblocks = (size_t)g.G * mgroups * g.polys * (g.form == GEMM_BSK ? c->hc.kb : c->hc.k) * (c->hc.n / 32);
-            if (g.form == GEMM_BSK) hipLaunchKernelGGL((k_scalar_gemm_mfma<P, false, GemmBskForm>), dim3((uint32_t)pblocks), dim3(256), 0, c->stream, g.in, g.idx, (const int8_t *)g.W, g.oidx,
+            if (g.form == GEMM_BSK) hipLaunchKernelGGL((k_scalar_gemm_mfma<P, false, GemmBskForm, RES...>), dim3((uint32_t)pblocks), dim3(256), 0, c->stream, g.in, g.idx, (const int8_t *)g.W, g.oidx,
                                                        nullptr, nullptr, g.out, c->dc, g.G, g.M, g.mtiles, g.ksteps, g.obase, g.polys, GemmUnits{g.in_unit, g.out_unit, 0u});
-            else hipLaunchKernelGGL((k_scalar_gemm_mfma<P, false, GemmYForm>), dim3((uint32_t)pblocks), dim3(256), 0, c->stream, g.in, g.idx, (const int8_t *)g.W, g.oidx,
+            else hipLaunchKernelGGL((k_scalar_gemm_mfma<P, false, GemmYForm, RES...>), dim3((uint32_t)pblocks), dim3(256), 0, c->stream, g.in, g.idx, (const int8_t *)g.W, g.oidx,
                                     nullptr, nullptr, g.out, c->dc, g.G, g.M, g.mtiles, g.ksteps, g.obase, g.polys, GemmUnits{g.in_unit, g.out_unit, 0u});
             return;
         }
     }
     const size_t blocks = (size_t)g.G * mgroups * g.polys * c->hc.k * (c->hc.n / 32);
-    hipLaunchKernelGGL((k_scalar_gemm_mfma<P, ABS>), dim3((uint32_t)blocks), dim3(256), 0, c->stream, g.in, g.idx, (const int8_t *)g.W, g.oidx, g.bias, g.bidx, g.out,
+    hipLaunchKernelGGL((k_scalar_gemm_mfma<P, ABS, RES...>), dim3((uint32_t)blocks), dim3(256), 0, c->stream, g.in, g.idx, (const int8_t *)g.W, g.oidx, g.bias, g.bidx, g.out,
                        c->dc, g.G, g.M, g.mtiles, g.ksteps, g.obase, g.polys, GemmUnits{g.in_unit, g.out_unit, g.bias_unit});
 }
 template <bool ABS> static int launch_mfma_p(cn_ctx *c, const GemmLaunch &g) {
     if (g.form && (ABS || g.P > 2 || g.form > GEMM_Y || !g.in_unit || !g.out_unit)) return cn_fail(CN_ERR_ARG, "internal: pre-floor GEMM form %u", g.form);
+    if (g.res && g.P != 1) return cn_fail(CN_ERR_ARG, "internal: residual weights with %u planes", g.P);
     switch (g.P) {
-        case 1: launch_mfma<1, ABS>(c, g); break;
+        case 1: if (g.res) launch_mfma<1, ABS, GemmResidual>(c, g); else launch_mfma<1, ABS>(c, g); break;
         case 2: launch_mfma<2, ABS>(c, g); break;
         case 3: launch_mfma<3, ABS>(c, g); break;
         default: return cn_fail(CN_ERR_ARG, "internal: %u weight digit planes", g.P);
@@ -85,18 +86,19 @@
     else hipLaunchKernelGGL((k_digit_gemm<MT, 5>), dim3((uint32_t)blocks), dim3(256), 0, c->stream, g.in, g.in_unit, (const int32_t *)g.idx, (const double *)g.W,
                             (const int32_t *)g.oidx, (double *)g.S, c->dc, g.G, g.M, g.K, mtiles, g.Kp, g.Kw, ndg);
 }
-template <int P, int DG> static void launch_digit_mfma(cn_ctx *c, const DigitGemmLaunch &g, uint32_t ndg, size_t blocks) {
-    if (g.i32) hipLaunchKernelGGL((k_digit_gemm_mfma<P, DG, int32_t>), dim3((uint32_t)blocks), dim3(256), 0, c->stream, g.in, g.in_unit, (const int32_t *)g.idx, (const int8_t *)g.W,
+template <int P, int DG, class... RES> static void launch_digit_mfma(cn_ctx *c, const DigitGemmLaunch &g, uint32_t ndg, size_t blocks) {
+    if (g.i32) hipLaunchKernelGGL((k_digit_gemm_mfma<P, DG, int32_t, RES...>), dim3((uint32_t)blocks), dim3(256), 0, c->stream, g.in, g.in_unit, (const int32_t *)g.idx, (const int8_t *)g.W,
                                   (const int32_t *)g.oidx, (int32_t *)g.S, c->dc, g.G, g.M, g.mtiles, g.ksteps, ndg);
-    else hipLaunchKernelGGL((k_digit_gemm_mfma<P, DG>), dim3((uint32_t)blocks), dim3(256), 0, c->stream, g.in, g.in_unit, (const int32_t *)g.idx, (const int8_t *)g.W,
+    else hipLaunchKernelGGL((k_digit_gemm_mfma<P, DG, RES...>), dim3((uint32_t)blocks), dim3(256), 0, c->stream, g.in, g.in_unit, (const int32_t *)g.idx, (const int8_t *)g.W,
                             (const int32_t *)g.oidx, (double *)g.S, c->dc, g.G, g.M, g.mtiles, g.ksteps, ndg);
 }
 static int digit_gemm_mfma(cn_ctx *c, const DigitGemmLaunch &g, uint32_t ndmax) {
-    const uint32_t DG = digit_gemm_mfma_group(g.P), ndg = (ndmax + DG - 1) / DG, mgroups = (g.mtiles + 3) / 4;
+    if (g.res && g.P != 1) return cn_fail(CN_ERR_ARG, "internal: residual weights with %u planes", g.P);
+    const uint32_t DG = g.res ? DIGIT_GEMM_RES_GROUP : digit_gemm_mfma_group(g.P), ndg = (ndmax + DG - 1) / DG, mgroups = (g.mtiles + 3) / 4;
     const uint64_t blocks = (uint64_t)g.G * mgroups * c->hc.k * (c->hc.n / 32) * ndg;
     if ((c->hc.n & 255) || !g.ksteps || blocks >= (1ull << 31)) return cn_fail(CN_ERR_ARG, "internal: digit GEMM grid");
     switch (g.P) {
-        case 1: launch_digit_mfma<1, 3>(c, g, ndg, blocks); break;
+        case 1: if (g.res) launch_digit_mfma<1, DIGIT_GEMM_RES_GROUP, GemmResidual>(c, g, ndg, blocks); else launch_digit_mfma<1, 3>(c, g, ndg, blocks); break;
         case 2: launch_digit_mfma<2, 3>(c, g, ndg, blocks); break;
         case 3: launch_digit_mfma<3, 2>(c, g, ndg, blocks); break;
         default: return cn_fail(CN_ERR_ARG, "internal: %u weight digit planes", g.P);
diff --git a/cryptonets_amd/csrc/cn_policy.h b/cryptonets_amd/csrc/cn_policy.h
--- a/cryptonets_amd/csrc/cn_policy.h
+++ b/cryptonets_amd/csrc/cn_policy.h
@@ -42,6 +42,7 @@
     uint32_t K = 0, Kp = 0, G = 0, M = 0, MT = 0, lazy = 0;
     bool small = false, two = false, one = false, mfma = false;
     uint32_t P = 0, mtiles = 0, ksteps = 0;
+    bool res = false;
     bool dig = false, dig_mfma = false, dig_i32 = false; uint32_t dMT = 0, dKw = 0;
     size_t off_oidx = 0, off_bidx = 0, off_w = 0, off_dw = 0;
     uint64_t sum_abs_w = 0;
diff --git a/cryptonets_amd/csrc/cn_runtime.h b/cryptonets_amd/csrc/cn_runtime.h
--- a/cryptonets_amd/csrc/cn_runtime.h
+++ b/cryptonets_amd/csrc/cn_runtime.h
@@ -243,12 +243,13 @@
     uint32_t polys = 2;
     uint32_t order = 0;
     bool one = false;
+    bool res = false;
     uint32_t in_unit = 0, out_unit = 0, bias_unit = 0;
     uint32_t form = 0;
     static GemmLaunch of(const GemmLayout &L, const char *tables, uint32_t order) {
         return {.small = L.small, .two = L.two, .abs = false, .MT = L.MT, .in = nullptr, .idx = tables, .W = tables + L.off_w, .oidx = tables + L.off_oidx, .bias = nullptr,
                 .bidx = tables + L.off_bidx, .out = nullptr, .G = L.G, .M = L.M, .K = L.K, .lazy = L.lazy, .Kp = L.Kp, .obase = 0, .P = L.P, .mtiles = L.mtiles, .ksteps = L.ksteps,
-                .order = order, .one = L.one};
+                .order = order, .one = L.one, .res = L.res};
     }
     GemmLaunch &inputs(const uint64_t *base, uint32_t unit, uint32_t polys_) { in = base; in_unit = unit; polys = polys_; return *this; }
     GemmLaunch &gather(const void *rows) { idx = rows; return *this; }
@@ -264,10 +265,11 @@
     uint32_t G, M, K, Kp, Kw, MT;
     bool mfma = false; uint32_t P = 0, mtiles = 0, ksteps = 0;
     bool i32 = false;
+    bool res = false;
     static DigitGemmLaunch of(const GemmLayout &L, const char *tables, const uint64_t *in, size_t in_unit, const void *idx, void *S) {
         return {.in = in, .in_unit = in_unit, .idx = idx, .W = tables + (L.dig_mfma ? L.off_w : L.off_dw), .oidx = tables + L.off_oidx, .S = S, .G = L.G, .M = L.M, .K = L.K,
                 .Kp = L.Kp, .Kw = L.dKw, .MT = L.dMT, .mfma = L.dig_mfma, .P = L.dig_mfma ? L.P : 0, .mtiles = L.dig_mfma ? L.mtiles : 0, .ksteps = L.dig_mfma ? L.ksteps : 0,
-                .i32 = L.dig_i32};
+                .i32 = L.dig_i32, .res = L.dig_mfma && L.res};
     }
 };
 inline uint32_t digit_gemm_mfma_group(uint32_t P) { return P <= 2 ? 3u : 2u; }
```
